# rakhimovv/lvt

Measured on AMD Instinct MI355X. Metric: video-clips/sec/node (VQVAE+DSFVT train step, BAIR 64x64x16), higher is better.
Workload: dtype f32

## Files before the change

include/lvt_hip.h:

```cpp
#ifndef LVT_HIP_H
#define LVT_HIP_H
#include <stddef.h>
#include <stdint.h>
#ifdef __cplusplus
extern "C" {
#endif

#define LVT_OK            0
#define LVT_EINVAL      (-1)
#define LVT_EWORKSPACE  (-2)
#define LVT_ELAUNCH     (-3)
#define LVT_ENODEVICE   (-4)

const char *lvt_last_error(void);
int lvt_version(void);
int lvt_device_info(char *name, int name_len, int *cus, int *clock_khz, long long *hbm_bytes);

#define LVT_MATH_F32   (1 << 16)
#define LVT_MATH_F16X2 (1 << 18)
typedef struct { const float *a; const float *b; float *c; } lvt_amax_io;
int lvt_amax(const float *x, long long n, float *out, void *stream);
typedef struct { const float *x; long long n; float *out; } lvt_amax_entry;
int lvt_amax_multi(const lvt_amax_entry *entries, int n, void *stream);
int lvt_amax_merge(const float *a, const float *b, float *out, void *stream);
#define LVT_VQ_COARSE  (1 << 17)
#define LVT_VQ_GENERIC (1 << 22)

#define LVT_EPI_BIAS        1
#define LVT_EPI_RESIDUAL    2
#define LVT_EPI_RELU        4
#define LVT_EPI_TANH        8
#define LVT_EPI_MASK       16
#define LVT_EPI_ACCUM      32
#define LVT_EPI_PLANES     64
#define LVT_EPI_SIGMOID   128
#define LVT_EPI_PAD(n)    (((n) & 3) << 24)
#define LVT_EPI_PAD_OF(flags) (((flags) >> 24) & 3)
#define LVT_EPI_LEAKY       (1 << 11)
#define LVT_EPI_LEAKY_MASK  (1 << 12)
#define LVT_CAUSAL_KMAX   (1 << 8)
#define LVT_CAUSAL_KMIN   (1 << 9)
#define LVT_CAUSAL_TILE   (1 << 10)

typedef struct {
    int M, N, K;
    int ta, tb;
    const float *A; long long lda; int a_kb; long long a_skb;
    const float *B; long long ldb; int b_kb; long long b_skb;
    float *C;       long long ldc;
    int batch_outer, batch_inner;
    long long sA_o, sA_i, sB_o, sB_i, sC_o, sC_i;
    float alpha;
    int flags;
    const float *bias;
    const float *res;  long long ldr;
    const float *mask; long long ldm;
    int splits;
    float *a_colsum;
    long long c_plane;
    const float *a_amax, *b_amax;
    const float *a_amax2, *b_amax2;
    float *c_amax;
} lvt_gemm_desc;
size_t lvt_gemm_workspace_bytes(const lvt_gemm_desc *d);
int lvt_gemm_f32(const lvt_gemm_desc *d, void *workspace, size_t workspace_bytes, void *stream);

int lvt_vq_argmax_scores(const float *scores, long long rows, int K, long long ld, const float *codebook, int D,
                         long long *idx, void *stream);

typedef struct {
    int M, N, K;
    const void *A; long long lda; int a_planes; int a_kb; long long a_skb;
    const void *B; long long ldb;
    float *C; long long ldc;
    int batch_outer, batch_inner;
    long long sA_o, sA_i, sB_o, sB_i, sC_o, sC_i;
    float alpha;
    int flags;
    const float *bias;
    const float *res;  long long ldr;
    const float *mask; long long ldm;
    const float *a_amax, *b_amax;
    float *c_amax;
    void *Cp; long long ldcp; const float *cp_amax;
} lvt_gemm_p2_desc;
int lvt_gemm_p2_f32(const lvt_gemm_p2_desc *d, void *stream);
typedef struct { const float *src; void *dst; int rows, cols; long long ld_src, ld_dst; int transpose; const float *amax;
                 int batch; long long bs_src, bs_dst; } lvt_p2_pack_entry;
int lvt_p2_pack_multi(const lvt_p2_pack_entry *entries, int n, void *stream);

int lvt_gemm_smallm_f32(int M, int N, int K, int tb, const float *A, long long lda, const float *B,
                        long long ldb, float *C, long long ldc, int batch, long long sB, long long sC,
                        float alpha, int flags, const float *bias, const float *res, long long ldr,
                        const int *pos, long long c_pos, long long r_pos, void *stream);
size_t lvt_gemm_smallm_splitk_workspace_bytes(int M, int N, int splits);
int lvt_gemm_smallm_splitk_f32(int M, int N, int K, int splits, const float *A, long long lda, const float *B,
                               long long ldb, float *C, long long ldc, float alpha, int flags, const float *bias,
                               const float *res, long long ldr, const int *pos, long long c_pos, long long r_pos,
                               void *workspace, size_t workspace_bytes, void *stream);
int lvt_gemm_smallm_partial_f32(int M, int N, int K, int splits, const float *A, long long lda, const float *B,
                                long long ldb, void *workspace, size_t workspace_bytes, void *stream);
int lvt_splitsum_layernorm_fwd(const float *partials, int splits, int rows, int d, const float *bias, const float *res,
                               long long ldr, float *x_out, float eps, const float *w, const float *b, float *y,
                               void *stream);

typedef struct {
    int N, Ti, Hi, Wi, Ci;
    int To, Ho, Wo, Co;
    int Kt, Kh, Kw;
    int st, sh, sw;
    int pt, ph, pw;
} lvt_conv_geom;
int lvt_conv3d_pack_weight(const lvt_conv_geom *g, const float *w, int Ci_real, int Co_real,
                           float *wp, void *stream);
typedef struct { const float *w; float *dst; int kind, taps, Ci, Co, Ci_real, Co_real; } lvt_pack_entry;
int lvt_conv3d_pack_weights_multi(const lvt_pack_entry *entries, int n, void *stream);
#define LVT_CONV_WEIGHT_IMAGE (1 << 21)
typedef struct { const float *wp; int rows, cols; const float *amax; } lvt_weight_image_entry;
size_t lvt_conv3d_weight_image_bytes(int rows, int cols);
int lvt_conv3d_weight_images(const lvt_weight_image_entry *entries, int n, void *stream);
int lvt_conv3d_pack_weight_t(const lvt_conv_geom *g, const float *w, int Ci_real, int Co_real,
                             float *wt, void *stream);
int lvt_conv3d_uses_patch_kernel(const lvt_conv_geom *g, int flags);
int lvt_conv3d_fwd_uses_parity_kernel(const lvt_conv_geom *g, int flags);
int lvt_conv3d_pack_weight_parity(const lvt_conv_geom *g, const float *w, int Ci_real, int Co_real,
                                  float *wq, void *stream);
int lvt_conv3d_fwd_parity(const lvt_conv_geom *g, const float *x, const float *wq, const float *bias,
                          const float *res, const float *mask, float *y, int flags, const lvt_amax_io *ax,
        void *stream);
int lvt_conv3d_fwd(const lvt_conv_geom *g, const float *x, const float *wp, const float *bias,
                   const float *res, const float *mask, float *y, int flags, const lvt_amax_io *ax,
        void *stream);
int lvt_conv3d_bwd_data_uses_phase_kernel(const lvt_conv_geom *g, int flags);
int lvt_conv3d_pack_weight_phases(const lvt_conv_geom *g, const float *w, int Ci_real, int Co_real,
                                  float *wph, void *stream);
int lvt_conv3d_bwd_data_phases(const lvt_conv_geom *g, const float *dy, const float *wph, const float *bias,
                               const float *res, const float *mask, float *dx, int flags, const lvt_amax_io *ax,
        void *stream);
int lvt_conv3d_bwd_data(const lvt_conv_geom *g, const float *dy, const float *wp, const float *bias,
                        const float *res, const float *mask, float *dx, int flags, const lvt_amax_io *ax,
        void *stream);
size_t lvt_conv3d_bwd_weight_workspace_bytes(const lvt_conv_geom *g);
int lvt_conv3d_bwd_weight_fuses_bias(const lvt_conv_geom *g, int flags);
#define LVT_WGRAD_DB_OF_X (1 << 20)
int lvt_conv3d_bwd_weight(const lvt_conv_geom *g, const float *x, const float *dy, float *dw, float *db,
                          int Ci_real, int Co_real, int flags, const lvt_amax_io *ax, void *workspace,
                          size_t workspace_bytes, void *stream);
int lvt_convt4_fwd(const float *x, const float *w, const float *bias, int N, int Hi, int Wi, int Ci, int Cr,
                   int act_tanh, float *y, int flags, const lvt_amax_io *ax, void *stream);
int lvt_convt4_fwd_act(const float *x, const float *w, const float *bias, int N, int Hi, int Wi, int Ci, int Cr,
                       int act, float *y, int flags, const lvt_amax_io *ax, void *stream);
size_t lvt_colsum_workspace_bytes(long long M, int N);
int lvt_colsum(const float *g, long long M, int N, long long ld, float *out, void *workspace,
               size_t workspace_bytes, void *stream);

size_t lvt_vq_nearest_workspace_bytes(long long rows, int num, int KC);
size_t lvt_vq_nearest_generic_workspace_bytes(int num, int D, int KC);
int lvt_vq_nearest(const float *z, long long rows, int ldz, int num, int D, int KC,
                   const float *codebooks, long long *idx, int P, int flags, void *workspace, size_t workspace_bytes,
                   void *stream);
int lvt_vq_gather(const long long *idx, const float *codebooks, long long rows, int num, int D, int KC,
                  int P, float *out, int ldo, void *stream);
size_t lvt_vq_ema_workspace_bytes(long long rows, int num, int D, int KC);
int lvt_vq_ema_accumulate(const long long *idx, const float *z, long long rows, int ldz, int num, int D,
                          int KC, int P, float *stats, void *workspace, size_t workspace_bytes,
                          void *stream);
int lvt_vq_ema_finalize(const float *stats, int num, int D, int KC, float decay, float eps,
                        float *running_size, float *running_sum, float *weight, void *stream);
int lvt_vq_restart_candidates(const float *z, long long rows_local, int ldz, int num, int D, int KC, int P, int rank,
                              int world, unsigned long long seed, const long long *pass, int shared_index, float *cand,
                              void *stream);
int lvt_vq_ema_finalize_restart(const float *stats, const float *cand, int num, int D, int KC, float decay, float eps,
                                float threshold, float *running_size, float *running_sum, float *weight, float *health,
                                long long *restarts_total, long long *pass, void *stream);

int lvt_to_channels_last(const float *in, int B, int C, long long R, int ldo, int mode, const float *a,
                         const float *s, float *out, float *out_amax, void *stream);
int lvt_to_channels_first(const float *in, int B, int C, long long R, int ldi, int mode, const float *a,
                          const float *s, float lo, float hi, float *out, void *stream);

size_t lvt_reduce_workspace_bytes(void);
int lvt_mse_fwd(const float *a, const float *b, long long n, double denom, float scale, float *out,
                void *workspace, size_t workspace_bytes, void *stream);
int lvt_mse_bwd(const float *a, const float *b, long long n, double denom, float scale,
                const float *gout_dev, const float *add, int tanh_of_a, float *out, float *out_amax, void *stream);
int lvt_l1_fwd(const float *a, const float *b, long long n, double denom, float scale, float *out,
               void *workspace, size_t workspace_bytes, void *stream);
int lvt_l1_bwd(const float *a, const float *b, long long n, double denom, float scale,
               const float *gout_dev, const float *add, int tanh_of_a, float *out, float *out_amax, void *stream);
int lvt_tanh_bwd(const float *g, const float *y, long long n, float *out, float *out_amax, void *stream);
int lvt_sigmoid_bwd(const float *g, const float *y, long long n, float *out, float *out_amax, void *stream);
int lvt_axpy(const float *x, const float *add, long long n, const float *alpha_dev, float alpha,
             float *out, void *stream);
int lvt_add_periodic(float *x, const float *table, long long rows, int P, int d, void *stream);

int lvt_layernorm_fwd(const float *x, long long rows, int d, float eps, const float *w, const float *b,
                      float *y, float *mean, float *rstd, float *y_amax, const float *w_amax, const float *b_amax,
                      void *stream);
int lvt_layernorm_fwd_p2(const float *x, long long rows, int d, float eps, const float *w, const float *b,
                         float *y, void *yp, float *mean, float *rstd, float *y_amax, const float *w_amax,
                         const float *b_amax, void *stream);
size_t lvt_layernorm_bwd_workspace_bytes(int d);
int lvt_layernorm_bwd(const float *dy, const float *x, const float *mean, const float *rstd,
                      const float *w, long long rows, int d, const float *add, float *dx, float *dw,
                      float *db, float *dx_amax, void *workspace, size_t workspace_bytes, void *stream);

int lvt_attn_softmax_fwd(float *scores, int B, int H, int S, float temper, const float *dt,
                         const float *dh, const float *dw, int bt, int bh, int bw, int masked, float fill,
                         void *stream);
int lvt_attn_softmax_bwd(const float *P, float *dP, int B, int H, int S, float temper, int bt, int bh,
                         int bw, float *G, float *ddt, float *ddh, float *ddw, void *stream);

int lvt_attn_fwd(const float *q, const float *k, const float *v, int B, int H, int S, int da, float temper,
                 const float *dt, const float *dh, const float *dw, int bt, int bh, int bw, int masked, float fill,
                 float *P, float *o, void *stream);

int lvt_attn_planes_supported(int S, int da, int bt, int bh, int bw);
int lvt_attn_fwd_planes(const void *qkv_planes, long long plane_stride, long long operand_stride, int B, int H, int S, int da,
                        float temper, const float *dt, const float *dh, const float *dw, int bt, int bh, int bw, int masked,
                        float fill, float *P, float *o, float *o_amax, void *stream);
size_t lvt_attn_bwd_planes_workspace_bytes(int B, int H, int S, int bt, int bh, int bw);
int lvt_attn_bwd_planes(const void *qkv_planes, long long plane_stride, long long operand_stride, const void *do_planes,
                        const float *P, const float *o, int B, int H, int S, int da, float temper, int bt, int bh, int bw,
                        int masked, float *dq, float *dk, float *dv, float *ddt, float *ddh, float *ddw, float *d_amax,
                        void *workspace, size_t workspace_bytes, void *stream);

int lvt_attn_flash_supported(int S, int da, int bt, int bh, int bw);
int lvt_attn_fwd_flash(const float *q, const float *k, const float *v, long long ld, int B, int H, int S, int da,
                       float temper, const float *dt, const float *dh, const float *dw, int bt, int bh, int bw,
                       int masked, float fill, float *o, float *stats, float *o_amax, void *stream);
size_t lvt_attn_bwd_flash_workspace_bytes(int B, int H, int S, int bt, int bh, int bw);
int lvt_attn_bwd_flash(const float *q, const float *k, const float *v, const float *d_o, long long ld, const float *stats,
                       const float *o, int B, int H, int S, int da, float temper, const float *dt, const float *dh, const float *dw,
                       int bt, int bh, int bw, int masked, float fill, float *dq, float *dk, float *dv, float *ddt,
                       float *ddh, float *ddw, float *d_amax, void *workspace, size_t workspace_bytes, void *stream);

int lvt_attn_decode(const float *q, long long ldq, const float *Kc, const float *Vc, int B, int H, int S, int da, int qi,
                    float temper, const float *dt, const float *dh, const float *dw, int bt, int bh, int bw,
                    float *o, const int *pos, long long q_pos, void *stream);
int lvt_attn_decode_blocks(const float *q, long long ldq, const float *Kc, const float *Vc, int B, int H, int da, int qi,
                           float temper, const float *dt, const float *dh, const float *dw, int st, int sh, int sw,
                           int bt, int bh, int bw, float *o, const int *pos, long long q_pos, void *stream);

int lvt_decode_gather_codes(const long long *codes, const long long *nb, const int *pos, int rows, int S1, int taps,
                            long long *out, void *stream);
int lvt_decode_commit(const long long *drawn, int rows, int S1, long long *codes, int *pos, void *stream);

int lvt_sample_categorical(const float *logits, long long rows, int V, float temp, const float *u,
                           long long *out, long long out_stride, float *probs, const int *pos, long long u_pos,
                           void *stream);

int lvt_embbag_fwd(const long long *idx, long long bstride, int P, long long rows, int nslots,
                   const int *slot_off, const int *tab_row, const float *table, int D, const float *bias,
                   const float *btable, const long long *bindex, float *out, void *stream);
#define LVT_ONEHOT_DENSE (1 << 19)
size_t lvt_onehot_tn_workspace_bytes(int nslots, int V, int N, long long rows);
int lvt_onehot_tn_is_gather(int nslots, int V, int N, long long ldb, const float *dout, int flags);
int lvt_onehot_tn_gemm(const long long *idx, int nslots, int V, const int *slot_off, long long bstride,
                       long long pstride, int P, long long rows, const float *dout, long long ldb, int N,
                       float *out, int flags, const float *dout_amax, void *workspace, size_t workspace_bytes,
                       void *stream);
int lvt_permute3(const float *in, long long s0, long long s1, long long s2, int n0, int n1, int n2,
                 float *out, void *stream);

int lvt_row_gather(const float *x, const long long *perm, long long B, int S, int d, float *out, void *stream);

int lvt_slice_context(const long long *video, int B, int T, int nc, int H, int W, const int *abc, int st, int sh,
                      int sw, int kt, int kh, int kw, int n_prime, long long pad_value, long long *ctx,
                      long long *slice, long long *slice_idx, unsigned char *ignore, void *stream);

size_t lvt_xent_workspace_bytes(void);
int lvt_xent_fwd(const float *logits, const long long *target, long long tstride_b, long long tstride_pos,
                 int P, long long rows, int V, long long ignore, float scale, float *row_loss, float *lse,
                 float *loss, float *count, void *workspace, size_t workspace_bytes, void *stream);
int lvt_xent_bwd(const float *logits, const long long *target, long long tstride_b, long long tstride_pos,
                 int P, long long rows, int V, long long ignore, const float *lse, const float *count,
                 const float *gout, float scale, float *dlogits, float *dl_amax, void *stream);

typedef struct {
    float *p; const float *g; float *s0; float *s1;
    long long n; float lr; float wd;
} lvt_opt_entry;
int lvt_adam_step(const lvt_opt_entry *entries, int n, float beta1, float beta2, float eps, int step,
                  void *stream);
int lvt_rmsprop_step(const lvt_opt_entry *entries, int n, float alpha, float eps, float momentum,
                     void *stream);

typedef struct { const float *g; long long n; } lvt_grad_entry;
typedef struct {
    float norm;
    float coef;
    int skip;
    int reserved;
} lvt_clip_record;
long long lvt_grad_sqnorm_partials(const lvt_grad_entry *entries, int n);
int lvt_grad_sqnorm(const lvt_grad_entry *entries, int n, double *partials, long long n_partials, void *stream);
int lvt_grad_clip_coef(const double *partials, long long n_partials, float max_norm, lvt_clip_record *record,
                       long long *skipped, void *stream);
int lvt_adam_step_scaled(const lvt_opt_entry *entries, int n, float beta1, float beta2, float eps, int step,
                         const lvt_clip_record *gscale, float clamp, void *stream);
int lvt_rmsprop_step_scaled(const lvt_opt_entry *entries, int n, float alpha, float eps, float momentum,
                            const lvt_clip_record *gscale, float clamp, void *stream);

#define LVT_BN_RUNNING  1
#define LVT_BN_UPDATE   2
#define LVT_BN_UNBIASED 4
#define LVT_BN_COUNT    8
#define LVT_BN_TRAIN    16
size_t lvt_bn_workspace_bytes(long long M, int Cp);
int lvt_bn_stats(const float *y, long long M, int Cp, float *stats, void *workspace, size_t workspace_bytes, void *stream);
int lvt_bn_finalize(const float *stats, int nranks, long long count, int C, int Cp, const float *gamma, const float *beta,
                    float *running_mean, float *running_var, long long *num_batches_tracked, float momentum, float eps,
                    int flags, float *scale, float *shift, float *saved, void *stream);
int lvt_bn_apply(const float *y, const float *res, long long M, int Cp, const float *scale, const float *shift, int flags,
                 float *out, float *out_amax, void *stream);
int lvt_bn_bwd_reduce(const float *g, const float *y, long long M, int Cp, const float *saved, float *sums, void *workspace,
                      size_t workspace_bytes, void *stream);
int lvt_bn_bwd_apply(const float *g, const float *y, long long M, int Cp, const float *scale, const float *saved,
                     const float *sums, long long n, int flags, float *dy, float *dy_amax, void *stream);
typedef struct {
    const float *w; float *w_out; int outer, Co, inner, Cp;
    const float *gamma, *beta, *running_mean, *running_var; float eps;
    float *bias_out; float *w_amax;
} lvt_bn_fold_entry;
int lvt_bn_fold(const lvt_bn_fold_entry *entries, int n, void *stream);


int lvt_pool2x2(const float *x, int N, int H, int W, int Cp, float scale, const float *mask, int mask_flags, float *out,
                float *out_amax, void *stream);
int lvt_upsample2x2(const float *x, int N, int H, int W, int Cp, float scale, const float *mask, int mask_flags, float *out,
                    float *out_amax, void *stream);

int lvt_pixel_shuffle2(const float *x, int N, int H, int W, int C, int act, float *out, float *out_amax, void *stream);
int lvt_pixel_unshuffle2(const float *g, int N, int H, int W, int C, float *out, float *out_amax, void *stream);

#ifdef __cplusplus
}
#endif
#endif
```

lvt_amd/csrc/elementwise.hip:

```cpp
#include "lvt_common.h"

static inline int grid_for(long long n, int per_block, int cap = 8192) {
    long long b = lvt_cdiv(n, per_block);
    if (b < 1) b = 1;
    return (int)(b < cap ? b : cap);
}

__device__ __forceinline__ float wave_sum(float v) {
#pragma unroll
    for (int off = 32; off >= 1; off >>= 1) v += __shfl_xor(v, off);
    return v;
}
__device__ __forceinline__ float wave_max(float v) {
#pragma unroll
    for (int off = 32; off >= 1; off >>= 1) v = fmaxf(v, __shfl_xor(v, off));
    return v;
}

__global__ void lvt_to_channels_last_kernel(const float *__restrict__ in, int B, int C, long long R, int ldo,
                                            int mode, const float *__restrict__ a, const float *__restrict__ s,
                                            float *__restrict__ out, float *__restrict__ out_amax) {
    __shared__ float amax_scratch[4];
    float am = 0.f;
    const long long total = (long long)B * R * ldo;
    for (long long i = (long long)blockIdx.x * blockDim.x + threadIdx.x; i < total;
         i += (long long)gridDim.x * blockDim.x) {
        const int c = i % ldo; const long long t = i / ldo;
        const long long r = t % R; const long long b = t / R;
        float v = 0.f;
        if (c < C) {
            v = in[(b * C + c) * R + r];
            if (mode == 1) v = (v - a[c]) / s[c];
        }
        out[i] = v;
        am = fmaxf(am, lvt_absf(v));
    }
    if (out_amax) lvt_block_amax_commit(am, out_amax, amax_scratch);
}
__global__ void lvt_to_channels_first_kernel(const float *__restrict__ in, int B, int C, long long R, int ldi,
                                             int mode, const float *__restrict__ a, const float *__restrict__ s,
                                             float lo, float hi, float *__restrict__ out) {
    const long long total = (long long)B * C * R;
    for (long long i = (long long)blockIdx.x * blockDim.x + threadIdx.x; i < total;
         i += (long long)gridDim.x * blockDim.x) {
        const long long r = i % R; const long long t = i / R;
        const int c = t % C; const long long b = t / C;
        float v = in[(b * R + r) * ldi + c];
        if (mode == 2) { v = v * s[c] + a[c]; v = fminf(fmaxf(v, lo), hi); }
        out[i] = v;
    }
}

extern "C" int lvt_to_channels_last(const float *in, int B, int C, long long R, int ldo, int mode, const float *a,
                                    const float *s, float *out, float *out_amax, void *stream) {
    LVT_REQUIRE(in && out && B > 0 && C > 0 && R > 0 && ldo >= C, "to_channels_last: bad args");
    LVT_REQUIRE(mode == 0 || (a && s), "to_channels_last: affine tables missing");
    hipLaunchKernelGGL(lvt_to_channels_last_kernel, dim3(grid_for((long long)B * R * ldo, 256, out_amax ? 2048 : 8192)), dim3(256), 0,
                       (hipStream_t)stream, in, B, C, R, ldo, mode, a, s, out, out_amax);
    LVT_CHECK_LAUNCH("lvt_to_channels_last_kernel");
    return LVT_OK;
}
extern "C" int lvt_to_channels_first(const float *in, int B, int C, long long R, int ldi, int mode, const float *a,
                                     const float *s, float lo, float hi, float *out, void *stream) {
    LVT_REQUIRE(in && out && B > 0 && C > 0 && R > 0 && ldi >= C, "to_channels_first: bad args");
    LVT_REQUIRE(mode == 0 || (a && s), "to_channels_first: affine tables missing");
    hipLaunchKernelGGL(lvt_to_channels_first_kernel, dim3(grid_for((long long)B * C * R, 256)), dim3(256), 0,
                       (hipStream_t)stream, in, B, C, R, ldi, mode, a, s, lo, hi, out);
    LVT_CHECK_LAUNCH("lvt_to_channels_first_kernel");
    return LVT_OK;
}

#define RED_BLOCKS 1024
template <int L1>
__global__ void lvt_sqdiff_partial_kernel(const float *__restrict__ a, const float *__restrict__ b, long long n4,
                                          float *__restrict__ partial) {
    __shared__ float red[256];
    float s = 0.f;
    for (long long i = (long long)blockIdx.x * blockDim.x + threadIdx.x; i < n4;
         i += (long long)gridDim.x * blockDim.x) {
        const float4 x = reinterpret_cast<const float4 *>(a)[i];
        const float4 y = reinterpret_cast<const float4 *>(b)[i];
        const float d0 = x.x - y.x, d1 = x.y - y.y, d2 = x.z - y.z, d3 = x.w - y.w;
        if (L1) s += (fabsf(d0) + fabsf(d1)) + (fabsf(d2) + fabsf(d3));
        else s += (d0 * d0 + d1 * d1) + (d2 * d2 + d3 * d3);
    }
    red[threadIdx.x] = s;
    __syncthreads();
    for (int k = 128; k > 0; k >>= 1) {
        if (threadIdx.x < k) red[threadIdx.x] += red[threadIdx.x + k];
        __syncthreads();
    }
    if (threadIdx.x == 0) partial[blockIdx.x] = red[0];
}
__global__ void lvt_scalar_finish_kernel(const float *__restrict__ partial, int n, float scale,
                                         const float *__restrict__ denom_dev, float *__restrict__ out) {
    __shared__ double red[256];
    double s = 0.0;
    for (int i = threadIdx.x; i < n; i += 256) s += (double)partial[i];
    red[threadIdx.x] = s;
    __syncthreads();
    for (int k = 128; k > 0; k >>= 1) {
        if (threadIdx.x < k) red[threadIdx.x] += red[threadIdx.x + k];
        __syncthreads();
    }
    if (threadIdx.x == 0) {
        double v = red[0] * (double)scale;
        if (denom_dev) v /= (double)fmaxf(denom_dev[0], 1.0f);
        out[0] = (float)v;
    }
}
extern "C" size_t lvt_reduce_workspace_bytes(void) { return (size_t)RED_BLOCKS * sizeof(float) * 2; }

extern "C" int lvt_mse_fwd(const float *a, const float *b, long long n, double denom, float scale, float *out,
                           void *workspace, size_t workspace_bytes, void *stream) {
    LVT_REQUIRE(a && b && out && n > 0 && n % 4 == 0 && denom > 0, "mse_fwd: bad args");
    LVT_REQUIRE(workspace && workspace_bytes >= lvt_reduce_workspace_bytes(), "mse_fwd: workspace");
    hipStream_t s = (hipStream_t)stream;
    const int blocks = grid_for(n / 4, 256 * 4, RED_BLOCKS);
    hipLaunchKernelGGL(lvt_sqdiff_partial_kernel<0>, dim3(blocks), dim3(256), 0, s, a, b, n / 4, (float *)workspace);
    LVT_CHECK_LAUNCH("lvt_sqdiff_partial_kernel");
    hipLaunchKernelGGL(lvt_scalar_finish_kernel, dim3(1), dim3(256), 0, s, (const float *)workspace, blocks,
                       (float)((double)scale / denom), (const float *)nullptr, out);
    LVT_CHECK_LAUNCH("lvt_scalar_finish_kernel");
    return LVT_OK;
}
extern "C" int lvt_l1_fwd(const float *a, const float *b, long long n, double denom, float scale, float *out,
                          void *workspace, size_t workspace_bytes, void *stream) {
    LVT_REQUIRE(a && b && out && n > 0 && n % 4 == 0 && denom > 0, "l1_fwd: bad args");
    LVT_REQUIRE(workspace && workspace_bytes >= lvt_reduce_workspace_bytes(), "l1_fwd: workspace");
    hipStream_t s = (hipStream_t)stream;
    const int blocks = grid_for(n / 4, 256 * 4, RED_BLOCKS);
    hipLaunchKernelGGL(lvt_sqdiff_partial_kernel<1>, dim3(blocks), dim3(256), 0, s, a, b, n / 4, (float *)workspace);
    LVT_CHECK_LAUNCH("lvt_sqdiff_partial_kernel<l1>");
    hipLaunchKernelGGL(lvt_scalar_finish_kernel, dim3(1), dim3(256), 0, s, (const float *)workspace, blocks,
                       (float)((double)scale / denom), (const float *)nullptr, out);
    LVT_CHECK_LAUNCH("lvt_scalar_finish_kernel");
    return LVT_OK;
}

template <int L1>
__global__ void lvt_mse_bwd_kernel(const float *__restrict__ a, const float *__restrict__ b, long long n4, float c,
                                   const float *__restrict__ gout, const float *__restrict__ add, int tanh_of_a,
                                   float *__restrict__ out, float *__restrict__ out_amax) {
    __shared__ float amax_scratch[4];
    float am = 0.f;
    const float g = (gout ? gout[0] : 1.0f) * c;
    for (long long i = (long long)blockIdx.x * blockDim.x + threadIdx.x; i < n4;
         i += (long long)gridDim.x * blockDim.x) {
        const float4 x = reinterpret_cast<const float4 *>(a)[i];
        const float4 y = reinterpret_cast<const float4 *>(b)[i];
        float4 r = make_float4(x.x - y.x, x.y - y.y, x.z - y.z, x.w - y.w);
        if (L1) r = make_float4((float)((r.x > 0.f) - (r.x < 0.f)), (float)((r.y > 0.f) - (r.y < 0.f)), (float)((r.z > 0.f) - (r.z < 0.f)),
                                (float)((r.w > 0.f) - (r.w < 0.f)));
        r.x *= g; r.y *= g; r.z *= g; r.w *= g;
        if (tanh_of_a) {
            r.x *= 1.f - x.x * x.x; r.y *= 1.f - x.y * x.y; r.z *= 1.f - x.z * x.z; r.w *= 1.f - x.w * x.w;
        }
        if (add) {
            const float4 z = reinterpret_cast<const float4 *>(add)[i];
            r.x += z.x; r.y += z.y; r.z += z.z; r.w += z.w;
        }
        reinterpret_cast<float4 *>(out)[i] = r;
        am = fmaxf(am, fmaxf(fmaxf(lvt_absf(r.x), lvt_absf(r.y)), fmaxf(lvt_absf(r.z), lvt_absf(r.w))));
    }
    if (out_amax) lvt_block_amax_commit(am, out_amax, amax_scratch);
}
extern "C" int lvt_mse_bwd(const float *a, const float *b, long long n, double denom, float scale,
                           const float *gout_dev, const float *add, int tanh_of_a, float *out, float *out_amax, void *stream) {
    LVT_REQUIRE(a && b && out && n > 0 && n % 4 == 0 && denom > 0, "mse_bwd: bad args");
    hipLaunchKernelGGL(lvt_mse_bwd_kernel<0>, dim3(grid_for(n / 4, 256, out_amax ? 2048 : 8192)), dim3(256), 0, (hipStream_t)stream, a, b,
                       n / 4, (float)(2.0 * (double)scale / denom), gout_dev, add, tanh_of_a, out, out_amax);
    LVT_CHECK_LAUNCH("lvt_mse_bwd_kernel");
    return LVT_OK;
}
extern "C" int lvt_l1_bwd(const float *a, const float *b, long long n, double denom, float scale,
                          const float *gout_dev, const float *add, int tanh_of_a, float *out, float *out_amax, void *stream) {
    LVT_REQUIRE(a && b && out && n > 0 && n % 4 == 0 && denom > 0, "l1_bwd: bad args");
    hipLaunchKernelGGL(lvt_mse_bwd_kernel<1>, dim3(grid_for(n / 4, 256, out_amax ? 2048 : 8192)), dim3(256), 0, (hipStream_t)stream, a, b,
                       n / 4, (float)((double)scale / denom), gout_dev, add, tanh_of_a, out, out_amax);
    LVT_CHECK_LAUNCH("lvt_mse_bwd_kernel<l1>");
    return LVT_OK;
}

__global__ void lvt_axpy_kernel(const float *__restrict__ x, const float *__restrict__ add, long long n,
                                const float *__restrict__ alpha_dev, float alpha, float *__restrict__ out) {
    const float a = alpha * (alpha_dev ? alpha_dev[0] : 1.0f);
    for (long long i = (long long)blockIdx.x * blockDim.x + threadIdx.x; i < n;
         i += (long long)gridDim.x * blockDim.x)
        out[i] = a * x[i] + (add ? add[i] : 0.f);
}
extern "C" int lvt_axpy(const float *x, const float *add, long long n, const float *alpha_dev, float alpha,
                        float *out, void *stream) {
    LVT_REQUIRE(x && out && n > 0, "axpy: bad args");
    hipLaunchKernelGGL(lvt_axpy_kernel, dim3(grid_for(n, 256)), dim3(256), 0, (hipStream_t)stream, x, add, n,
                       alpha_dev, alpha, out);
    LVT_CHECK_LAUNCH("lvt_axpy_kernel");
    return LVT_OK;
}

__global__ void lvt_tanh_bwd_kernel(const float *__restrict__ g, const float *__restrict__ y, long long n4,
                                    float *__restrict__ out, float *__restrict__ out_amax) {
    __shared__ float amax_scratch[4];
    float am = 0.f;
    for (long long i = (long long)blockIdx.x * blockDim.x + threadIdx.x; i < n4;
         i += (long long)gridDim.x * blockDim.x) {
        const float4 a = reinterpret_cast<const float4 *>(g)[i];
        const float4 t = reinterpret_cast<const float4 *>(y)[i];
        const float4 r = make_float4(a.x * (1.f - t.x * t.x), a.y * (1.f - t.y * t.y), a.z * (1.f - t.z * t.z), a.w * (1.f - t.w * t.w));
        reinterpret_cast<float4 *>(out)[i] = r;
        am = fmaxf(am, fmaxf(fmaxf(lvt_absf(r.x), lvt_absf(r.y)), fmaxf(lvt_absf(r.z), lvt_absf(r.w))));
    }
    if (out_amax) lvt_block_amax_commit(am, out_amax, amax_scratch);
}
extern "C" int lvt_tanh_bwd(const float *g, const float *y, long long n, float *out, float *out_amax, void *stream) {
    LVT_REQUIRE(g && y && out && n > 0 && n % 4 == 0, "tanh_bwd: bad args");
    hipLaunchKernelGGL(lvt_tanh_bwd_kernel, dim3(grid_for(n / 4, 256, out_amax ? 2048 : 8192)), dim3(256), 0, (hipStream_t)stream, g, y,
                       n / 4, out, out_amax);
    LVT_CHECK_LAUNCH("lvt_tanh_bwd_kernel");
    return LVT_OK;
}

__global__ void lvt_sigmoid_bwd_kernel(const float *__restrict__ g, const float *__restrict__ y, long long n4,
                                       float *__restrict__ out, float *__restrict__ out_amax) {
    __shared__ float amax_scratch[4];
    float am = 0.f;
    for (long long i = (long long)blockIdx.x * blockDim.x + threadIdx.x; i < n4;
         i += (long long)gridDim.x * blockDim.x) {
        const float4 a = reinterpret_cast<const float4 *>(g)[i];
        const float4 t = reinterpret_cast<const float4 *>(y)[i];
        const float4 r = make_float4(a.x * (t.x * (1.f - t.x)), a.y * (t.y * (1.f - t.y)), a.z * (t.z * (1.f - t.z)), a.w * (t.w * (1.f - t.w)));
        reinterpret_cast<float4 *>(out)[i] = r;
        am = fmaxf(am, fmaxf(fmaxf(lvt_absf(r.x), lvt_absf(r.y)), fmaxf(lvt_absf(r.z), lvt_absf(r.w))));
    }
    if (out_amax) lvt_block_amax_commit(am, out_amax, amax_scratch);
}
extern "C" int lvt_sigmoid_bwd(const float *g, const float *y, long long n, float *out, float *out_amax, void *stream) {
    LVT_REQUIRE(g && y && out && n > 0 && n % 4 == 0, "sigmoid_bwd: bad args");
    hipLaunchKernelGGL(lvt_sigmoid_bwd_kernel, dim3(grid_for(n / 4, 256, out_amax ? 2048 : 8192)), dim3(256), 0, (hipStream_t)stream, g, y,
                       n / 4, out, out_amax);
    LVT_CHECK_LAUNCH("lvt_sigmoid_bwd_kernel");
    return LVT_OK;
}

__global__ void lvt_add_periodic_kernel(float *__restrict__ x, const float *__restrict__ table, long long rows,
                                        int P, int d4) {
    const long long total = rows * d4;
    for (long long i = (long long)blockIdx.x * blockDim.x + threadIdx.x; i < total;
         i += (long long)gridDim.x * blockDim.x) {
        const long long r = i / d4; const int c = i % d4;
        float4 v = reinterpret_cast<float4 *>(x)[i];
        const float4 t = reinterpret_cast<const float4 *>(table)[(r % P) * d4 + c];
        v.x += t.x; v.y += t.y; v.z += t.z; v.w += t.w;
        reinterpret_cast<float4 *>(x)[i] = v;
    }
}
extern "C" int lvt_add_periodic(float *x, const float *table, long long rows, int P, int d, void *stream) {
    LVT_REQUIRE(x && table && rows > 0 && P > 0 && d % 4 == 0, "add_periodic: bad args");
    hipLaunchKernelGGL(lvt_add_periodic_kernel, dim3(grid_for(rows * (d / 4), 256)), dim3(256), 0,
                       (hipStream_t)stream, x, table, rows, P, d / 4);
    LVT_CHECK_LAUNCH("lvt_add_periodic_kernel");
    return LVT_OK;
}

#define LN_MAXV 4
__device__ __forceinline__ float ln_bound(const float *w_amax, const float *b_amax, int d) {
    return fmaf(*w_amax, sqrtf((float)(d - 1)), *b_amax) * (1.0f + 0x1p-20f);
}
__device__ __forceinline__ float ln_mix_lo(unsigned h, float k, float c) {
    float r;
    asm("v_fma_mix_f32 %0, %1, %2, %3 op_sel:[0,0,0] op_sel_hi:[1,0,0]" : "=v"(r) : "v"(h), "v"(k), "v"(c));
    return r;
}
__device__ __forceinline__ float ln_mix_hi(unsigned h, float k, float c) {
    float r;
    asm("v_fma_mix_f32 %0, %1, %2, %3 op_sel:[1,0,0] op_sel_hi:[1,0,0]" : "=v"(r) : "v"(h), "v"(k), "v"(c));
    return r;
}
typedef float ln_f32x2 __attribute__((ext_vector_type(2)));
typedef _Float16 ln_f16x2 __attribute__((ext_vector_type(2)));
__device__ __forceinline__ void ln_split_pair(float a, float b, float s, unsigned &ph, unsigned &pl) {
    const ln_f32x2 v = {a, b};
    ph = __builtin_bit_cast(unsigned, __builtin_convertvector(v * s, ln_f16x2));
    const ln_f32x2 t2 = v * (s * 2048.f);
    const ln_f32x2 r = {ln_mix_lo(ph, -2048.f, t2.x), ln_mix_hi(ph, -2048.f, t2.y)};
    pl = __builtin_bit_cast(unsigned, __builtin_convertvector(r, ln_f16x2));
}
template <int P2>
__global__ void lvt_layernorm_fwd_kernel(const float *__restrict__ x, long long rows, int d, float eps,
                                         const float *__restrict__ w, const float *__restrict__ b,
                                         float *__restrict__ y, float *__restrict__ mean_out,
                                         float *__restrict__ rstd_out, float *__restrict__ y_amax,
                                         const float *__restrict__ w_amax, const float *__restrict__ b_amax,
                                         char *__restrict__ yimg) {
    __shared__ float amax_scratch[4];
    const int lane = threadIdx.x & 63;
    const int d4 = d / 4;
    float am = 0.f;
    float ps = 1.f;
    if (P2) {
        int un = 0;
        ps = lvt_f16_scale_bits(__float_as_uint(ln_bound(w_amax, b_amax, d)), un);
    }
    if (y_amax && w_amax) {
        if (blockIdx.x == 0 && threadIdx.x == 0) *y_amax = ln_bound(w_amax, b_amax, d);
        y_amax = nullptr;
    }
    for (long long row = ((long long)blockIdx.x * blockDim.x + threadIdx.x) >> 6; row < rows;
         row += ((long long)gridDim.x * blockDim.x) >> 6) {
        const float4 *xp = reinterpret_cast<const float4 *>(x + row * d);
        float4 v[LN_MAXV];
        float s = 0.f;
#pragma unroll
        for (int i = 0; i < LN_MAXV; ++i) {
            const int c = lane + 64 * i;
            v[i] = c < d4 ? xp[c] : make_float4(0.f, 0.f, 0.f, 0.f);
            s += (v[i].x + v[i].y) + (v[i].z + v[i].w);
        }
        const float mean = wave_sum(s) / d;
        float q = 0.f;
#pragma unroll
        for (int i = 0; i < LN_MAXV; ++i) {
            if (lane + 64 * i < d4) {
                const float a0 = v[i].x - mean, a1 = v[i].y - mean, a2 = v[i].z - mean, a3 = v[i].w - mean;
                q += (a0 * a0 + a1 * a1) + (a2 * a2 + a3 * a3);
            }
        }
        const float rstd = 1.0f / sqrtf(wave_sum(q) / d + eps);
        float4 *yp = reinterpret_cast<float4 *>(y + row * d);
#pragma unroll
        for (int i = 0; i < LN_MAXV; ++i) {
            const int c = lane + 64 * i;
            if (c < d4) {
                const float4 ww = reinterpret_cast<const float4 *>(w)[c];
                const float4 bb = reinterpret_cast<const float4 *>(b)[c];
                float4 o;
                o.x = (v[i].x - mean) * rstd * ww.x + bb.x; o.y = (v[i].y - mean) * rstd * ww.y + bb.y;
                o.z = (v[i].z - mean) * rstd * ww.z + bb.z; o.w = (v[i].w - mean) * rstd * ww.w + bb.w;
                yp[c] = o;
                if (P2) {
                    uint2 ph, pl;
                    ln_split_pair(o.x, o.y, ps, ph.x, pl.x);
                    ln_split_pair(o.z, o.w, ps, ph.y, pl.y);
                    char *ip = yimg + (long long)row * d * 4 + (c >> 3) * 128 + (c & 7) * 8;
                    *reinterpret_cast<uint2 *>(ip) = ph;
                    *reinterpret_cast<uint2 *>(ip + 64) = pl;
                }
                am = fmaxf(am, fmaxf(fmaxf(lvt_absf(o.x), lvt_absf(o.y)), fmaxf(lvt_absf(o.z), lvt_absf(o.w))));
            }
        }
        if (lane == 0 && mean_out) { mean_out[row] = mean; rstd_out[row] = rstd; }
    }
    if (y_amax) lvt_block_amax_commit(am, y_amax, amax_scratch);
}
#define LN_FWD_MAX_BLOCKS 16384
extern "C" int lvt_layernorm_fwd(const float *x, long long rows, int d, float eps, const float *w, const float *b,
                                 float *y, float *mean, float *rstd, float *y_amax, const float *w_amax, const float *b_amax,
                                 void *stream) {
    LVT_REQUIRE(x && w && b && y && rows > 0 && d % 4 == 0 && d <= 256 * LN_MAXV, "layernorm_fwd: bad args (d=%d)", d);
    LVT_REQUIRE(!w_amax == !b_amax, "layernorm_fwd: w_amax and b_amax come together");
    hipLaunchKernelGGL(lvt_layernorm_fwd_kernel<0>, dim3(grid_for(rows, 4, (y_amax && !w_amax) ? 2048 : LN_FWD_MAX_BLOCKS)), dim3(256), 0,
                       (hipStream_t)stream, x, rows, d, eps, w, b, y, mean, rstd, y_amax, w_amax, b_amax, (char *)nullptr);
    LVT_CHECK_LAUNCH("lvt_layernorm_fwd_kernel");
    return LVT_OK;
}
extern "C" int lvt_layernorm_fwd_p2(const float *x, long long rows, int d, float eps, const float *w, const float *b,
                                    float *y, void *yp, float *mean, float *rstd, float *y_amax, const float *w_amax,
                                    const float *b_amax, void *stream) {
    LVT_REQUIRE(x && w && b && y && yp && rows > 0 && d % 32 == 0 && d <= 256 * LN_MAXV, "layernorm_fwd_p2: bad args (d=%d)", d);
    LVT_REQUIRE(y_amax && w_amax && b_amax, "layernorm_fwd_p2: the image is scaled by the a-priori bound: y_amax, w_amax, b_amax are required");
    LVT_REQUIRE(((uintptr_t)yp & 127) == 0, "layernorm_fwd_p2: the image must be 128-byte aligned");
    hipLaunchKernelGGL(lvt_layernorm_fwd_kernel<1>, dim3(grid_for(rows, 4, LN_FWD_MAX_BLOCKS)), dim3(256), 0,
                       (hipStream_t)stream, x, rows, d, eps, w, b, y, mean, rstd, y_amax, w_amax, b_amax, (char *)yp);
    LVT_CHECK_LAUNCH("lvt_layernorm_fwd_kernel<p2>");
    return LVT_OK;
}

#define LN_BWD_BLOCKS 512
#define LN_BWD_ROWS 1
__global__ __launch_bounds__(256) void lvt_layernorm_bwd_kernel(
    const float *__restrict__ dy, const float *__restrict__ x, const float *__restrict__ mean,
    const float *__restrict__ rstd, const float *__restrict__ w, long long rows, int d, const float *__restrict__ add,
    float *__restrict__ dx, float *__restrict__ pdw, float *__restrict__ pdb, float *__restrict__ dx_amax) {
    __shared__ float amax_scratch[4];
    float am = 0.f;
    __shared__ float sdw[4][256 * LN_MAXV];
    __shared__ float sdb[4][256 * LN_MAXV];
    const int lane = threadIdx.x & 63, wave = threadIdx.x >> 6;
    const int d4 = d / 4;
    float4 adw[LN_MAXV], adb[LN_MAXV];
#pragma unroll
    for (int i = 0; i < LN_MAXV; ++i) { adw[i] = make_float4(0.f, 0.f, 0.f, 0.f); adb[i] = adw[i]; }
    const long long rows_per_block = lvt_cdiv(rows, gridDim.x);
    const long long r0 = blockIdx.x * rows_per_block;
    const long long r1 = min(rows, r0 + rows_per_block);
    for (long long row0 = r0 + wave; row0 < r1; row0 += 4 * LN_BWD_ROWS) {
        float4 xh[LN_BWD_ROWS][LN_MAXV], gw[LN_BWD_ROWS][LN_MAXV], zv[LN_BWD_ROWS][LN_MAXV];
        float rs[LN_BWD_ROWS], s1[LN_BWD_ROWS], s2[LN_BWD_ROWS];
#pragma unroll
        for (int u = 0; u < LN_BWD_ROWS; ++u) {
            const long long row = row0 + 4 * u;
            if (row >= r1) continue;
            if (add) {
#pragma unroll
                for (int i = 0; i < LN_MAXV; ++i)
                    if (lane + 64 * i < d4) zv[u][i] = reinterpret_cast<const float4 *>(add + row * d)[lane + 64 * i];
            }
            const float m = mean[row];
            rs[u] = rstd[row];
            const float4 *xp = reinterpret_cast<const float4 *>(x + row * d);
            const float4 *gp = reinterpret_cast<const float4 *>(dy + row * d);
            s1[u] = 0.f; s2[u] = 0.f;
#pragma unroll
            for (int i = 0; i < LN_MAXV; ++i) {
                const int c = lane + 64 * i;
                if (c < d4) {
                    const float4 xv = xp[c], gv = gp[c], ww = reinterpret_cast<const float4 *>(w)[c];
                    const float r = rs[u];
                    xh[u][i] = make_float4((xv.x - m) * r, (xv.y - m) * r, (xv.z - m) * r, (xv.w - m) * r);
                    gw[u][i] = make_float4(gv.x * ww.x, gv.y * ww.y, gv.z * ww.z, gv.w * ww.w);
                    const float4 h = xh[u][i], g = gw[u][i];
                    s1[u] += (g.x + g.y) + (g.z + g.w);
                    s2[u] += (g.x * h.x + g.y * h.y) + (g.z * h.z + g.w * h.w);
                    adw[i].x += gv.x * h.x; adw[i].y += gv.y * h.y; adw[i].z += gv.z * h.z; adw[i].w += gv.w * h.w;
                    adb[i].x += gv.x; adb[i].y += gv.y; adb[i].z += gv.z; adb[i].w += gv.w;
                }
            }
        }
#pragma unroll
        for (int u = 0; u < LN_BWD_ROWS; ++u) {
            const long long row = row0 + 4 * u;
            if (row >= r1) continue;
            const float m1 = wave_sum(s1[u]) / d, m2 = wave_sum(s2[u]) / d;
            float4 *op = reinterpret_cast<float4 *>(dx + row * d);
#pragma unroll
            for (int i = 0; i < LN_MAXV; ++i) {
                const int c = lane + 64 * i;
                if (c < d4) {
                    const float4 h = xh[u][i], g = gw[u][i];
                    const float r = rs[u];
                    float4 o;
                    o.x = r * (g.x - m1 - h.x * m2); o.y = r * (g.y - m1 - h.y * m2);
                    o.z = r * (g.z - m1 - h.z * m2); o.w = r * (g.w - m1 - h.w * m2);
                    if (add) {
                        const float4 z = zv[u][i];
                        o.x += z.x; o.y += z.y; o.z += z.z; o.w += z.w;
                    }
                    op[c] = o;
                    am = fmaxf(am, fmaxf(fmaxf(lvt_absf(o.x), lvt_absf(o.y)), fmaxf(lvt_absf(o.z), lvt_absf(o.w))));
                }
            }
        }
    }
    if (dx_amax) lvt_block_amax_commit(am, dx_amax, amax_scratch);
#pragma unroll
    for (int i = 0; i < LN_MAXV; ++i) {
        const int c = lane + 64 * i;
        if (c < d4) {
            reinterpret_cast<float4 *>(sdw[wave])[c] = adw[i];
            reinterpret_cast<float4 *>(sdb[wave])[c] = adb[i];
        }
    }
    __syncthreads();
    for (int c = threadIdx.x; c < d; c += 256) {
        pdw[(long long)blockIdx.x * d + c] = ((sdw[0][c] + sdw[1][c]) + sdw[2][c]) + sdw[3][c];
        pdb[(long long)blockIdx.x * d + c] = ((sdb[0][c] + sdb[1][c]) + sdb[2][c]) + sdb[3][c];
    }
}
__global__ __launch_bounds__(256) void lvt_rowsum_partials_kernel(const float *__restrict__ partial0, const float *__restrict__ partial1,
                                                                  int nblk, int n, float *__restrict__ out0, float *__restrict__ out1) {
    __shared__ float red[256];
    const float *partial = blockIdx.y ? partial1 : partial0;
    float *out = blockIdx.y ? out1 : out0;
    constexpr int cols = 8, RL = 256 / cols;
    const int c = blockIdx.x * cols + (threadIdx.x % cols);
    const int rl = threadIdx.x / cols;
    float s0 = 0.f, s1 = 0.f, s2 = 0.f, s3 = 0.f;
    if (c < n) {
        int b = rl;
        for (; b + 3 * RL < nblk; b += 4 * RL) {
            s0 += partial[(long long)b * n + c]; s1 += partial[(long long)(b + RL) * n + c];
            s2 += partial[(long long)(b + 2 * RL) * n + c]; s3 += partial[(long long)(b + 3 * RL) * n + c];
        }
        for (; b < nblk; b += RL) s0 += partial[(long long)b * n + c];
    }
    float s = (s0 + s1) + (s2 + s3);
    red[threadIdx.x] = s;
    __syncthreads();
    if (rl == 0 && c < n) {
        for (int k = 1; k < RL; ++k) s += red[k * cols + threadIdx.x];
        out[c] = s;
    }
}
extern "C" size_t lvt_layernorm_bwd_workspace_bytes(int d) { return (size_t)2 * LN_BWD_BLOCKS * d * sizeof(float); }
extern "C" int lvt_layernorm_bwd(const float *dy, const float *x, const float *mean, const float *rstd,
                                 const float *w, long long rows, int d, const float *add, float *dx, float *dw,
                                 float *db, float *dx_amax, void *workspace, size_t workspace_bytes, void *stream) {
    LVT_REQUIRE(dy && x && mean && rstd && w && dx && dw && db && rows > 0 && d % 4 == 0 && d <= 256 * LN_MAXV,
                "layernorm_bwd: bad args");
    LVT_REQUIRE(workspace && workspace_bytes >= lvt_layernorm_bwd_workspace_bytes(d), "layernorm_bwd: workspace");
    hipStream_t s = (hipStream_t)stream;
    int blocks = (int)(lvt_cdiv(rows, 8) < LN_BWD_BLOCKS ? lvt_cdiv(rows, 8) : LN_BWD_BLOCKS);
    const long long rpb = lvt_cdiv(rows, blocks);
    blocks = (int)lvt_cdiv(rows, rpb);
    float *pdw = (float *)workspace, *pdb = pdw + (size_t)LN_BWD_BLOCKS * d;
    hipLaunchKernelGGL(lvt_layernorm_bwd_kernel, dim3(blocks), dim3(256), 0, s, dy, x, mean, rstd, w, rows, d, add,
                       dx, pdw, pdb, dx_amax);
    LVT_CHECK_LAUNCH("lvt_layernorm_bwd_kernel");
    hipLaunchKernelGGL(lvt_rowsum_partials_kernel, dim3((d + 7) / 8, 2), dim3(256), 0, s, (const float *)pdw, (const float *)pdb,
                       blocks, d, dw, db);
    LVT_CHECK_LAUNCH("lvt_rowsum_partials_kernel");
    return LVT_OK;
}

struct SliceGeom { int B, T, nc, H, W, st, sh, sw, kt, kh, kw, n_prime, t, h, w, Tc, Hc, Wc; long long pad; };
__global__ void lvt_slice_context_kernel(const long long *__restrict__ video, const int *__restrict__ abc, SliceGeom g,
                                         long long *__restrict__ ctx, long long *__restrict__ slice,
                                         long long *__restrict__ slice_idx, unsigned char *__restrict__ ignore) {
    const long long n_ctx = (long long)g.B * g.nc * g.Tc * g.Hc * g.Wc;
    const long long n_sl = (long long)g.B * g.nc * g.t * g.h * g.w;
    const long long n_ig = (long long)g.B * g.t * g.h * g.w;
    const long long total = n_ctx + n_sl + n_ig + g.B;
    for (long long i = (long long)blockIdx.x * blockDim.x + threadIdx.x; i < total; i += (long long)gridDim.x * blockDim.x) {
        if (i < n_ctx) {
            long long r = i;
            const int ow = r % g.Wc; r /= g.Wc;
            const int oh = r % g.Hc; r /= g.Hc;
            const int ot = r % g.Tc; r /= g.Tc;
            const int ch = r % g.nc; const int b = r / g.nc;
            const int a = abc[3 * b], bo = abc[3 * b + 1], c = abc[3 * b + 2];
            const int ti = ot - g.kt / 2 + a, hi = oh - g.kh / 2 + bo, wi = ow - g.kw / 2 + c;
            long long v = g.pad;
            if ((unsigned)ti < (unsigned)g.T && (unsigned)hi < (unsigned)g.H && (unsigned)wi < (unsigned)g.W) {
                const int mine = ((ti % g.st) * g.sh + (hi % g.sh)) * g.sw + (wi % g.sw);
                if (mine < (a * g.sh + bo) * g.sw + c)
                    v = video[((((long long)b * g.T + ti) * g.nc + ch) * g.H + hi) * g.W + wi];
            }
            ctx[i] = v;
        } else if (i < n_ctx + n_sl) {
            long long r = i - n_ctx;
            const int wi = r % g.w; r /= g.w;
            const int hi = r % g.h; r /= g.h;
            const int ti = r % g.t; r /= g.t;
            const int ch = r % g.nc; const int b = r / g.nc;
            const int a = abc[3 * b], bo = abc[3 * b + 1], c = abc[3 * b + 2];
            slice[i - n_ctx] = video[((((long long)b * g.T + ti * g.st + a) * g.nc + ch) * g.H + hi * g.sh + bo) * g.W + wi * g.sw + c];
        } else if (i < n_ctx + n_sl + n_ig) {
            long long r = i - n_ctx - n_sl;
            r /= (long long)g.h * g.w;
            const int ti = r % g.t; const int b = r / g.t;
            ignore[i - n_ctx - n_sl] = (ti * g.st + abc[3 * b]) < g.n_prime ? 1 : 0;
        } else {
            const int b = (int)(i - n_ctx - n_sl - n_ig);
            slice_idx[b] = (abc[3 * b] * g.sh + abc[3 * b + 1]) * g.sw + abc[3 * b + 2];
        }
    }
}
extern "C" int lvt_slice_context(const long long *video, int B, int T, int nc, int H, int W, const int *abc, int st, int sh,
                                 int sw, int kt, int kh, int kw, int n_prime, long long pad_value, long long *ctx,
                                 long long *slice, long long *slice_idx, unsigned char *ignore, void *stream) {
    LVT_REQUIRE(video && abc && ctx && slice && slice_idx && ignore, "slice_context: null pointer");
    LVT_REQUIRE(B > 0 && nc > 0 && st > 0 && sh > 0 && sw > 0 && T % st == 0 && H % sh == 0 && W % sw == 0 &&
                kt > 0 && kh > 0 && kw > 0, "slice_context: bad geometry");
    SliceGeom g;
    g.B = B; g.T = T; g.nc = nc; g.H = H; g.W = W; g.st = st; g.sh = sh; g.sw = sw; g.kt = kt; g.kh = kh; g.kw = kw;
    g.n_prime = n_prime; g.pad = pad_value;
    g.t = T / st; g.h = H / sh; g.w = W / sw;
    g.Tc = 2 * (kt / 2) + (g.t - 1) * st + 1; g.Hc = 2 * (kh / 2) + (g.h - 1) * sh + 1; g.Wc = 2 * (kw / 2) + (g.w - 1) * sw + 1;
    const long long total = (long long)B * nc * g.Tc * g.Hc * g.Wc + (long long)B * (nc + 1) * g.t * g.h * g.w + B;
    const int blocks = (int)(lvt_cdiv(total, 256) < 4096 ? lvt_cdiv(total, 256) : 4096);
    hipLaunchKernelGGL(lvt_slice_context_kernel, dim3(blocks), dim3(256), 0, (hipStream_t)stream, video, abc, g, ctx, slice,
                       slice_idx, ignore);
    LVT_CHECK_LAUNCH("lvt_slice_context_kernel");
    return LVT_OK;
}

__global__ void lvt_row_gather_kernel(const float *__restrict__ x, const long long *__restrict__ perm, long long B, int S,
                                      int d4, float *__restrict__ out) {
    const long long total = B * S * d4;
    for (long long i = (long long)blockIdx.x * blockDim.x + threadIdx.x; i < total; i += (long long)gridDim.x * blockDim.x) {
        const int c = i % d4; const long long r = i / d4;
        const int s = r % S; const long long b = r / S;
        reinterpret_cast<float4 *>(out)[i] = reinterpret_cast<const float4 *>(x)[(b * S + perm[s]) * d4 + c];
    }
}
extern "C" int lvt_row_gather(const float *x, const long long *perm, long long B, int S, int d, float *out, void *stream) {
    LVT_REQUIRE(x && perm && out && B > 0 && S > 0 && d > 0 && d % 4 == 0 && lvt_aligned16(x) && lvt_aligned16(out),
                "row_gather: bad args");
    const long long total = B * S * (d / 4);
    const int blocks = (int)(lvt_cdiv(total, 256) < 8192 ? lvt_cdiv(total, 256) : 8192);
    hipLaunchKernelGGL(lvt_row_gather_kernel, dim3(blocks), dim3(256), 0, (hipStream_t)stream, x, perm, B, S, d / 4, out);
    LVT_CHECK_LAUNCH("lvt_row_gather_kernel");
    return LVT_OK;
}

__global__ __launch_bounds__(256) void lvt_amax_kernel(const float *__restrict__ x, long long n, float *__restrict__ out) {
    __shared__ float scratch[4];
    const long long n4 = n >> 2;
    float m = 0.f;
    if ((((uintptr_t)x) & 15) == 0) {
        float m1 = 0.f;
        long long i = (long long)blockIdx.x * blockDim.x + threadIdx.x;
        const long long step = (long long)gridDim.x * blockDim.x;
        for (; i + step < n4; i += 2 * step) {
            const float4 v = *reinterpret_cast<const float4 *>(x + i * 4), u = *reinterpret_cast<const float4 *>(x + (i + step) * 4);
            m = fmaxf(m, fmaxf(fmaxf(lvt_absf(v.x), lvt_absf(v.y)), fmaxf(lvt_absf(v.z), lvt_absf(v.w))));
            m1 = fmaxf(m1, fmaxf(fmaxf(lvt_absf(u.x), lvt_absf(u.y)), fmaxf(lvt_absf(u.z), lvt_absf(u.w))));
        }
        if (i < n4) {
            const float4 v = *reinterpret_cast<const float4 *>(x + i * 4);
            m = fmaxf(m, fmaxf(fmaxf(lvt_absf(v.x), lvt_absf(v.y)), fmaxf(lvt_absf(v.z), lvt_absf(v.w))));
        }
        m = fmaxf(m, m1);
        for (long long t = n4 * 4 + (long long)blockIdx.x * blockDim.x + threadIdx.x; t < n; t += step) m = fmaxf(m, lvt_absf(x[t]));
    } else {
        for (long long i = (long long)blockIdx.x * blockDim.x + threadIdx.x; i < n; i += (long long)gridDim.x * blockDim.x)
            m = fmaxf(m, lvt_absf(x[i]));
    }
    lvt_block_amax_commit(m, out, scratch);
}
struct AmaxTable { const float *x[64]; long long n[64]; float *out[64]; };
__global__ __launch_bounds__(256) void lvt_amax_multi_kernel(const AmaxTable t) {
    __shared__ float scratch[4];
    const float *x = t.x[blockIdx.y];
    const long long n = t.n[blockIdx.y], n4 = (((uintptr_t)x) & 15) == 0 ? n >> 2 : 0;
    float m = 0.f;
    for (long long i = (long long)blockIdx.x * blockDim.x + threadIdx.x; i < n4; i += (long long)gridDim.x * blockDim.x) {
        const float4 v = *reinterpret_cast<const float4 *>(x + i * 4);
        m = fmaxf(m, fmaxf(fmaxf(lvt_absf(v.x), lvt_absf(v.y)), fmaxf(lvt_absf(v.z), lvt_absf(v.w))));
    }
    for (long long i = n4 * 4 + (long long)blockIdx.x * blockDim.x + threadIdx.x; i < n; i += (long long)gridDim.x * blockDim.x)
        m = fmaxf(m, lvt_absf(x[i]));
    lvt_block_amax_commit(m, t.out[blockIdx.y], scratch);
}
extern "C" int lvt_amax_multi(const lvt_amax_entry *entries, int n, void *stream) {
    LVT_REQUIRE(entries && n > 0, "amax_multi: bad args");
    for (int base = 0; base < n; base += 64) {
        const int cnt = n - base < 64 ? n - base : 64;
        AmaxTable t;
        long long biggest = 0;
        for (int i = 0; i < cnt; ++i) {
            const lvt_amax_entry &e = entries[base + i];
            LVT_REQUIRE(e.x && e.out && e.n > 0, "amax_multi: bad entry %d", base + i);
            t.x[i] = e.x; t.n[i] = e.n; t.out[i] = e.out;
            if (e.n > biggest) biggest = e.n;
        }
        hipLaunchKernelGGL(lvt_amax_multi_kernel, dim3(grid_for(biggest / 4 + 1, 256 * 4, 64), cnt), dim3(256), 0, (hipStream_t)stream, t);
        LVT_CHECK_LAUNCH("lvt_amax_multi_kernel");
    }
    return LVT_OK;
}
__global__ void lvt_amax_merge_kernel(const float *a, const float *b, float *out) {
    float m = fmaxf(*out, *a);
    if (b) m = fmaxf(m, *b);
    *out = m;
}
extern "C" int lvt_amax_merge(const float *a, const float *b, float *out, void *stream) {
    LVT_REQUIRE(a && out, "amax_merge: bad args");
    hipLaunchKernelGGL(lvt_amax_merge_kernel, dim3(1), dim3(1), 0, (hipStream_t)stream, a, b, out);
    LVT_CHECK_LAUNCH("lvt_amax_merge_kernel");
    return LVT_OK;
}
extern "C" int lvt_amax(const float *x, long long n, float *out, void *stream) {
    LVT_REQUIRE(x && out && n > 0, "amax: bad args");
    hipLaunchKernelGGL(lvt_amax_kernel, dim3(grid_for(n / 4 + 1, 256 * 8, 1024)), dim3(256), 0, (hipStream_t)stream, x, n, out);
    LVT_CHECK_LAUNCH("lvt_amax_kernel");
    return LVT_OK;
}
```

lvt_amd/hip/binding.py:

```python
import ctypes as C
import os

import torch

_HERE = os.path.dirname(os.path.abspath(__file__))
_LIB_PATH = os.environ.get("LVT_HIP_LIB") or os.path.join(os.path.dirname(_HERE), "liblvt_hip.so")

EPI_BIAS, EPI_RESIDUAL, EPI_RELU, EPI_TANH, EPI_MASK, EPI_ACCUM, EPI_PLANES = 1, 2, 4, 8, 16, 32, 64
EPI_SIGMOID = 128
EPI_LEAKY, EPI_LEAKY_MASK = 1 << 11, 1 << 12


def epi_pad(n):
    if not 0 <= n <= 3:
        raise ValueError("epi_pad: 0..3 pad channels, got %r" % (n,))
    return n << 24
CAUSAL_KMAX, CAUSAL_KMIN, CAUSAL_TILE = 1 << 8, 1 << 9, 1 << 10
ABI_VERSION = 680
MATH_F32 = 1 << 16
MATH_F16X2 = 1 << 18
ONEHOT_DENSE = 1 << 19
WGRAD_DB_OF_X = 1 << 20
CONV_WEIGHT_IMAGE = 1 << 21
BN_RUNNING, BN_UPDATE, BN_UNBIASED, BN_COUNT, BN_TRAIN = 1, 2, 4, 8, 16


class LvtError(RuntimeError):
    pass


class GemmDesc(C.Structure):
    _fields_ = [
        ("M", C.c_int), ("N", C.c_int), ("K", C.c_int), ("ta", C.c_int), ("tb", C.c_int),
        ("A", C.c_void_p), ("lda", C.c_longlong), ("a_kb", C.c_int), ("a_skb", C.c_longlong),
        ("B", C.c_void_p), ("ldb", C.c_longlong), ("b_kb", C.c_int), ("b_skb", C.c_longlong),
        ("C", C.c_void_p), ("ldc", C.c_longlong),
        ("batch_outer", C.c_int), ("batch_inner", C.c_int),
        ("sA_o", C.c_longlong), ("sA_i", C.c_longlong), ("sB_o", C.c_longlong), ("sB_i", C.c_longlong),
        ("sC_o", C.c_longlong), ("sC_i", C.c_longlong),
        ("alpha", C.c_float), ("flags", C.c_int),
        ("bias", C.c_void_p), ("res", C.c_void_p), ("ldr", C.c_longlong),
        ("mask", C.c_void_p), ("ldm", C.c_longlong), ("splits", C.c_int),
        ("a_colsum", C.c_void_p), ("c_plane", C.c_longlong),
        ("a_amax", C.c_void_p), ("b_amax", C.c_void_p), ("a_amax2", C.c_void_p), ("b_amax2", C.c_void_p), ("c_amax", C.c_void_p),
    ]


class GemmP2Desc(C.Structure):
    _fields_ = [
        ("M", C.c_int), ("N", C.c_int), ("K", C.c_int),
        ("A", C.c_void_p), ("lda", C.c_longlong), ("a_planes", C.c_int), ("a_kb", C.c_int), ("a_skb", C.c_longlong),
        ("B", C.c_void_p), ("ldb", C.c_longlong),
        ("C", C.c_void_p), ("ldc", C.c_longlong),
        ("batch_outer", C.c_int), ("batch_inner", C.c_int),
        ("sA_o", C.c_longlong), ("sA_i", C.c_longlong), ("sB_o", C.c_longlong), ("sB_i", C.c_longlong),
        ("sC_o", C.c_longlong), ("sC_i", C.c_longlong),
        ("alpha", C.c_float), ("flags", C.c_int),
        ("bias", C.c_void_p), ("res", C.c_void_p), ("ldr", C.c_longlong),
        ("mask", C.c_void_p), ("ldm", C.c_longlong),
        ("a_amax", C.c_void_p), ("b_amax", C.c_void_p), ("c_amax", C.c_void_p),
        ("Cp", C.c_void_p), ("ldcp", C.c_longlong), ("cp_amax", C.c_void_p),
    ]


class P2PackEntry(C.Structure):
    _fields_ = [("src", C.c_void_p), ("dst", C.c_void_p), ("rows", C.c_int), ("cols", C.c_int), ("ld_src", C.c_longlong),
                ("ld_dst", C.c_longlong), ("transpose", C.c_int), ("amax", C.c_void_p),
                ("batch", C.c_int), ("bs_src", C.c_longlong), ("bs_dst", C.c_longlong)]


class AmaxEntry(C.Structure):
    _fields_ = [("x", C.c_void_p), ("n", C.c_longlong), ("out", C.c_void_p)]


class PackEntry(C.Structure):
    _fields_ = [("w", C.c_void_p), ("dst", C.c_void_p), ("kind", C.c_int), ("taps", C.c_int), ("Ci", C.c_int), ("Co", C.c_int),
                ("Ci_real", C.c_int), ("Co_real", C.c_int)]


class WeightImageEntry(C.Structure):
    _fields_ = [("wp", C.c_void_p), ("rows", C.c_int), ("cols", C.c_int), ("amax", C.c_void_p)]


class BnFoldEntry(C.Structure):
    _fields_ = [("w", C.c_void_p), ("w_out", C.c_void_p), ("outer", C.c_int), ("Co", C.c_int), ("inner", C.c_int),
                ("Cp", C.c_int), ("gamma", C.c_void_p), ("beta", C.c_void_p), ("running_mean", C.c_void_p),
                ("running_var", C.c_void_p), ("eps", C.c_float), ("bias_out", C.c_void_p), ("w_amax", C.c_void_p)]


class AmaxIO(C.Structure):
    _fields_ = [("a", C.c_void_p), ("b", C.c_void_p), ("c", C.c_void_p)]


class OptEntry(C.Structure):
    _fields_ = [("p", C.c_void_p), ("g", C.c_void_p), ("s0", C.c_void_p), ("s1", C.c_void_p),
                ("n", C.c_longlong), ("lr", C.c_float), ("wd", C.c_float)]


class GradEntry(C.Structure):
    _fields_ = [("g", C.c_void_p), ("n", C.c_longlong)]


CLIP_RECORD_BYTES = 16


class ConvGeom(C.Structure):
    _fields_ = [(n, C.c_int) for n in
                ("N", "Ti", "Hi", "Wi", "Ci", "To", "Ho", "Wo", "Co", "Kt", "Kh", "Kw",
                 "st", "sh", "sw", "pt", "ph", "pw")]

    def key(self):
        return tuple(getattr(self, n) for n, _ in self._fields_)


_lib = None


def _declare(lib):
    vp, ci, cll, cf, sz = C.c_void_p, C.c_int, C.c_longlong, C.c_float, C.c_size_t
    P = C.POINTER
    sigs = {
        "lvt_last_error": (C.c_char_p, []),
        "lvt_version": (ci, []),
        "lvt_device_info": (ci, [C.c_char_p, ci, P(ci), P(ci), P(cll)]),
        "lvt_gemm_workspace_bytes": (sz, [P(GemmDesc)]),
        "lvt_gemm_f32": (ci, [P(GemmDesc), vp, sz, vp]),
        "lvt_vq_argmax_scores": (ci, [vp, cll, ci, cll, vp, ci, vp, vp]),
        "lvt_gemm_p2_f32": (ci, [P(GemmP2Desc), vp]),
        "lvt_p2_pack_multi": (ci, [P(P2PackEntry), ci, vp]),
        "lvt_layernorm_fwd_p2": (ci, [vp, cll, ci, cf, vp, vp, vp, vp, vp, vp, vp, vp, vp, vp]),
        "lvt_gemm_smallm_f32": (ci, [ci, ci, ci, ci, vp, cll, vp, cll, vp, cll, ci, cll, cll, cf, ci, vp, vp, cll, vp, cll, cll, vp]),
        "lvt_gemm_smallm_splitk_workspace_bytes": (sz, [ci, ci, ci]),
        "lvt_gemm_smallm_splitk_f32": (ci, [ci, ci, ci, ci, vp, cll, vp, cll, vp, cll, cf, ci, vp, vp, cll, vp, cll, cll, vp, sz, vp]),
        "lvt_gemm_smallm_partial_f32": (ci, [ci, ci, ci, ci, vp, cll, vp, cll, vp, sz, vp]),
        "lvt_splitsum_layernorm_fwd": (ci, [vp, ci, ci, ci, vp, vp, cll, vp, cf, vp, vp, vp, vp]),
        "lvt_conv3d_pack_weight": (ci, [P(ConvGeom), vp, ci, ci, vp, vp]),
        "lvt_conv3d_pack_weight_t": (ci, [P(ConvGeom), vp, ci, ci, vp, vp]),
        "lvt_conv3d_uses_patch_kernel": (ci, [P(ConvGeom), ci]),
        "lvt_conv3d_fwd_uses_parity_kernel": (ci, [P(ConvGeom), ci]),
        "lvt_conv3d_pack_weight_parity": (ci, [P(ConvGeom), vp, ci, ci, vp, vp]),
        "lvt_amax": (ci, [vp, cll, vp, vp]),
        "lvt_amax_multi": (ci, [P(AmaxEntry), ci, vp]),
        "lvt_conv3d_pack_weights_multi": (ci, [P(PackEntry), ci, vp]),
        "lvt_conv3d_weight_image_bytes": (sz, [ci, ci]),
        "lvt_conv3d_weight_images": (ci, [P(WeightImageEntry), ci, vp]),
        "lvt_amax_merge": (ci, [vp, vp, vp, vp]),
        "lvt_conv3d_fwd_parity": (ci, [P(ConvGeom), vp, vp, vp, vp, vp, vp, ci, P(AmaxIO), vp]),
        "lvt_conv3d_fwd": (ci, [P(ConvGeom), vp, vp, vp, vp, vp, vp, ci, P(AmaxIO), vp]),
        "lvt_conv3d_bwd_data_uses_phase_kernel": (ci, [P(ConvGeom), ci]),
        "lvt_conv3d_pack_weight_phases": (ci, [P(ConvGeom), vp, ci, ci, vp, vp]),
        "lvt_conv3d_bwd_data_phases": (ci, [P(ConvGeom), vp, vp, vp, vp, vp, vp, ci, P(AmaxIO), vp]),
        "lvt_conv3d_bwd_data": (ci, [P(ConvGeom), vp, vp, vp, vp, vp, vp, ci, P(AmaxIO), vp]),
        "lvt_conv3d_bwd_weight_workspace_bytes": (sz, [P(ConvGeom)]),
        "lvt_conv3d_bwd_weight_fuses_bias": (ci, [P(ConvGeom), ci]),
        "lvt_conv3d_bwd_weight": (ci, [P(ConvGeom), vp, vp, vp, vp, ci, ci, ci, P(AmaxIO), vp, sz, vp]),
        "lvt_convt4_fwd": (ci, [vp, vp, vp, ci, ci, ci, ci, ci, ci, vp, ci, vp, vp]),
        "lvt_convt4_fwd_act": (ci, [vp, vp, vp, ci, ci, ci, ci, ci, ci, vp, ci, vp, vp]),
        "lvt_colsum_workspace_bytes": (sz, [cll, ci]),
        "lvt_colsum": (ci, [vp, cll, ci, cll, vp, vp, sz, vp]),
        "lvt_vq_nearest_workspace_bytes": (sz, [cll, ci, ci]),
        "lvt_vq_nearest_generic_workspace_bytes": (sz, [ci, ci, ci]),
        "lvt_vq_nearest": (ci, [vp, cll, ci, ci, ci, ci, vp, vp, ci, ci, vp, sz, vp]),
        "lvt_vq_gather": (ci, [vp, vp, cll, ci, ci, ci, ci, vp, ci, vp]),
        "lvt_vq_ema_workspace_bytes": (sz, [cll, ci, ci, ci]),
        "lvt_vq_ema_accumulate": (ci, [vp, vp, cll, ci, ci, ci, ci, ci, vp, vp, sz, vp]),
        "lvt_vq_ema_finalize": (ci, [vp, ci, ci, ci, cf, cf, vp, vp, vp, vp]),
        "lvt_vq_restart_candidates": (ci, [vp, cll, ci, ci, ci, ci, ci, ci, ci, C.c_ulonglong, vp, ci, vp, vp]),
        "lvt_vq_ema_finalize_restart": (ci, [vp, vp, ci, ci, ci, cf, cf, cf, vp, vp, vp, vp, vp, vp, vp]),
        "lvt_to_channels_last": (ci, [vp, ci, ci, cll, ci, ci, vp, vp, vp, vp, vp]),
        "lvt_to_channels_first": (ci, [vp, ci, ci, cll, ci, ci, vp, vp, cf, cf, vp, vp]),
        "lvt_reduce_workspace_bytes": (sz, []),
        "lvt_mse_fwd": (ci, [vp, vp, cll, C.c_double, cf, vp, vp, sz, vp]),
        "lvt_mse_bwd": (ci, [vp, vp, cll, C.c_double, cf, vp, vp, ci, vp, vp, vp]),
        "lvt_l1_fwd": (ci, [vp, vp, cll, C.c_double, cf, vp, vp, sz, vp]),
        "lvt_l1_bwd": (ci, [vp, vp, cll, C.c_double, cf, vp, vp, ci, vp, vp, vp]),
        "lvt_tanh_bwd": (ci, [vp, vp, cll, vp, vp, vp]),
        "lvt_sigmoid_bwd": (ci, [vp, vp, cll, vp, vp, vp]),
        "lvt_axpy": (ci, [vp, vp, cll, vp, cf, vp, vp]),
        "lvt_add_periodic": (ci, [vp, vp, cll, ci, ci, vp]),
        "lvt_layernorm_fwd": (ci, [vp, cll, ci, cf, vp, vp, vp, vp, vp, vp, vp, vp, vp]),
        "lvt_layernorm_bwd_workspace_bytes": (sz, [ci]),
        "lvt_layernorm_bwd": (ci, [vp, vp, vp, vp, vp, cll, ci, vp, vp, vp, vp, vp, vp, sz, vp]),
        "lvt_attn_softmax_fwd": (ci, [vp, ci, ci, ci, cf, vp, vp, vp, ci, ci, ci, ci, cf, vp]),
        "lvt_attn_softmax_bwd": (ci, [vp, vp, ci, ci, ci, cf, ci, ci, ci, vp, vp, vp, vp, vp]),
        "lvt_attn_fwd": (ci, [vp, vp, vp, ci, ci, ci, ci, cf, vp, vp, vp, ci, ci, ci, ci, cf, vp, vp, vp]),
        "lvt_attn_planes_supported": (ci, [ci, ci, ci, ci, ci]),
        "lvt_attn_fwd_planes": (ci, [vp, cll, cll, ci, ci, ci, ci, cf, vp, vp, vp, ci, ci, ci, ci, cf, vp, vp, vp, vp]),
        "lvt_attn_bwd_planes_workspace_bytes": (sz, [ci, ci, ci, ci, ci, ci]),
        "lvt_attn_bwd_planes": (ci, [vp, cll, cll, vp, vp, vp, ci, ci, ci, ci, cf, ci, ci, ci, ci, vp, vp, vp, vp, vp, vp, vp, vp, sz, vp]),
        "lvt_attn_flash_supported": (ci, [ci, ci, ci, ci, ci]),
        "lvt_attn_fwd_flash": (ci, [vp, vp, vp, cll, ci, ci, ci, ci, cf, vp, vp, vp, ci, ci, ci, ci, cf, vp, vp, vp, vp]),
        "lvt_attn_bwd_flash_workspace_bytes": (sz, [ci, ci, ci, ci, ci, ci]),
        "lvt_attn_bwd_flash": (ci, [vp, vp, vp, vp, cll, vp, vp, ci, ci, ci, ci, cf, vp, vp, vp, ci, ci, ci, ci, cf, vp, vp, vp, vp,
                                    vp, vp, vp, vp, sz, vp]),
        "lvt_attn_decode": (ci, [vp, cll, vp, vp, ci, ci, ci, ci, ci, cf, vp, vp, vp, ci, ci, ci, vp, vp, cll, vp]),
        "lvt_attn_decode_blocks": (ci, [vp, cll, vp, vp, ci, ci, ci, ci, cf, vp, vp, vp, ci, ci, ci, ci, ci, ci, vp, vp, cll, vp]),
        "lvt_decode_gather_codes": (ci, [vp, vp, vp, ci, ci, ci, vp, vp]),
        "lvt_decode_commit": (ci, [vp, ci, ci, vp, vp, vp]),
        "lvt_sample_categorical": (ci, [vp, cll, ci, cf, vp, vp, cll, vp, vp, cll, vp]),
        "lvt_embbag_fwd": (ci, [vp, cll, ci, cll, ci, P(ci), P(ci), vp, ci, vp, vp, vp, vp, vp]),
        "lvt_onehot_tn_workspace_bytes": (sz, [ci, ci, ci, cll]),
        "lvt_onehot_tn_is_gather": (ci, [ci, ci, ci, cll, vp, ci]),
        "lvt_onehot_tn_gemm": (ci, [vp, ci, ci, P(ci), cll, cll, ci, cll, vp, cll, ci, vp, ci, vp, vp, sz, vp]),
        "lvt_permute3": (ci, [vp, cll, cll, cll, ci, ci, ci, vp, vp]),
        "lvt_row_gather": (ci, [vp, vp, cll, ci, ci, vp, vp]),
        "lvt_slice_context": (ci, [vp, ci, ci, ci, ci, ci, vp, ci, ci, ci, ci, ci, ci, ci, cll, vp, vp, vp, vp, vp]),
        "lvt_xent_workspace_bytes": (sz, []),
        "lvt_xent_fwd": (ci, [vp, vp, cll, cll, ci, cll, ci, cll, cf, vp, vp, vp, vp, vp, sz, vp]),
        "lvt_xent_bwd": (ci, [vp, vp, cll, cll, ci, cll, ci, cll, vp, vp, vp, cf, vp, vp, vp]),
        "lvt_adam_step": (ci, [P(OptEntry), ci, cf, cf, cf, ci, vp]),
        "lvt_rmsprop_step": (ci, [P(OptEntry), ci, cf, cf, cf, vp]),
        "lvt_adam_step_scaled": (ci, [P(OptEntry), ci, cf, cf, cf, ci, vp, cf, vp]),
        "lvt_rmsprop_step_scaled": (ci, [P(OptEntry), ci, cf, cf, cf, vp, cf, vp]),
        "lvt_grad_sqnorm_partials": (cll, [P(GradEntry), ci]),
        "lvt_grad_sqnorm": (ci, [P(GradEntry), ci, vp, cll, vp]),
        "lvt_grad_clip_coef": (ci, [vp, cll, cf, vp, vp, vp]),
        "lvt_bn_workspace_bytes": (sz, [cll, ci]),
        "lvt_bn_stats": (ci, [vp, cll, ci, vp, vp, sz, vp]),
        "lvt_bn_finalize": (ci, [vp, ci, cll, ci, ci, vp, vp, vp, vp, vp, cf, cf, ci, vp, vp, vp, vp]),
        "lvt_bn_apply": (ci, [vp, vp, cll, ci, vp, vp, ci, vp, vp, vp]),
        "lvt_bn_bwd_reduce": (ci, [vp, vp, cll, ci, vp, vp, vp, sz, vp]),
        "lvt_bn_bwd_apply": (ci, [vp, vp, cll, ci, vp, vp, vp, cll, ci, vp, vp, vp]),
        "lvt_bn_fold": (ci, [P(BnFoldEntry), ci, vp]),
        "lvt_pool2x2": (ci, [vp, ci, ci, ci, ci, cf, vp, ci, vp, vp, vp]),
        "lvt_upsample2x2": (ci, [vp, ci, ci, ci, ci, cf, vp, ci, vp, vp, vp]),
        "lvt_pixel_shuffle2": (ci, [vp, ci, ci, ci, ci, ci, vp, vp, vp]),
        "lvt_pixel_unshuffle2": (ci, [vp, ci, ci, ci, ci, vp, vp, vp]),
    }
    for name, (res, args) in sigs.items():
        fn = getattr(lib, name)
        fn.restype = res
        fn.argtypes = args
    return sigs


def available():
    return os.path.exists(_LIB_PATH)


def lib():
    global _lib
    if _lib is None:
        if not os.path.exists(_LIB_PATH):
            raise LvtError("liblvt_hip.so not found at %s -- run `python -c 'import __graft_entry__ as g; "
                           "g.build()'` (or `make -C lvt_amd/csrc`); there is no CPU fallback" % _LIB_PATH)
        handle = C.CDLL(_LIB_PATH)
        handle.lvt_version.restype = C.c_int
        if handle.lvt_version() != ABI_VERSION:
            raise LvtError("liblvt_hip.so at %s has ABI version %d, this package binds version %d -- rebuild it "
                           "(`make -C lvt_amd/csrc`)" % (_LIB_PATH, handle.lvt_version(), ABI_VERSION))
        handle._lvt_sigs = _declare(handle)
        _lib = handle
    return _lib


MATH_MODES = ("f32", "bf16x3", "f16x2")
_math_mode = os.environ.get("LVT_MATH", "f16x2")
if _math_mode not in MATH_MODES:
    raise LvtError("LVT_MATH must be one of %s (got %r)" % (MATH_MODES, _math_mode))


def set_math_mode(mode):
    global _math_mode
    if mode not in MATH_MODES:
        raise LvtError("math mode must be one of %s (got %r)" % (MATH_MODES, mode))
    _math_mode = mode
    bump_epoch()


def get_math_mode():
    return _math_mode


def math_flag():
    return MATH_F32 if _math_mode == "f32" else (MATH_F16X2 if _math_mode == "f16x2" else 0)


def f16x2():
    return _math_mode == "f16x2"


_amax_pool, _amax_pos, _epoch = None, 0, 0
_wgen, _wlog = 0, {}
_WLOG_MAX = 64


def bump_epoch():
    global _epoch
    _epoch += 1
    _wlog.clear()


def amax_slot(device):
    global _amax_pool, _amax_pos
    if _amax_pool is None or _amax_pos >= _amax_pool.numel() or _amax_pool.device != device:
        _amax_pool, _amax_pos = torch.zeros(4096, dtype=torch.float32, device=device), 0
    s = _amax_pool[_amax_pos:_amax_pos + 1]
    _amax_pos += 1
    return s


def _extent(t):
    st = t.untyped_storage()
    key, lo = st.data_ptr(), t.data_ptr()
    span = 1
    for n, s in zip(t.shape, t.stride()):
        if n == 0:
            return key, lo, lo, False
        span += (n - 1) * s
    hi = lo + span * t.element_size()
    return key, lo, hi, lo <= key and hi >= key + st.nbytes()


def _note_write(t):
    global _wgen
    _wgen += 1
    key, lo, hi, whole = _extent(t)
    if whole:
        _wlog[key] = [_wgen, []]
    else:
        log = _wlog.setdefault(key, [0, []])
        log[1].append((_wgen, lo, hi))
        if len(log[1]) > _WLOG_MAX:
            log[0] = log[1].pop(0)[0]
    return key, lo, hi


def set_amax(t, slot, _ext=None):
    key, lo, hi = _ext if _ext is not None else _extent(t)[:3]
    t._lvt_amax = (slot, t._version, _epoch, t.data_ptr(), key, _wgen, lo, hi)
    return t


def drop_amax(t):
    t._lvt_amax = None
    _note_write(t)


AMAX_CHECK = bool(os.environ.get("LVT_AMAX_CHECK"))


def _checked(slot, t):
    if AMAX_CHECK and not torch.cuda.is_current_stream_capturing():
        have, real = float(slot), float(t.detach().abs().max()) if t.numel() else 0.0
        if not have >= real:
            raise LvtError("stale max |.| record: %g recorded, %g in the tensor of shape %s (an in-place kernel wrapper that "
                           "did not call binding.drop_amax?)" % (have, real, tuple(t.shape)))
    return slot


def _valid_amax(t):
    rec = getattr(t, "_lvt_amax", None)
    if rec is None or rec[1] != t._version or rec[2] != _epoch or rec[3] != t.data_ptr():
        return None
    log = _wlog.get(rec[4])
    if log is not None:
        gen = rec[5]
        if gen < log[0]:
            return None
        for g, lo, hi in reversed(log[1]):
            if g <= gen:
                break
            if lo < rec[7] and rec[6] < hi:
                return None
    return rec[0]


def new_amax(t):
    ext = _note_write(t)
    slot = amax_slot(t.device)
    set_amax(t, slot, ext)
    return slot


def amax_of(t):
    slot = _valid_amax(t)
    if slot is not None:
        return _checked(slot, t)
    base = t._base
    if base is not None:
        slot = _valid_amax(base)
        if slot is not None:
            return _checked(slot, t)
    src = t
    if not t.is_contiguous():
        if base is None or not base.is_contiguous():
            raise LvtError("amax_of: non-contiguous tensor without a contiguous base")
        src = base
    require(src)
    slot = amax_slot(src.device)
    check(lib().lvt_amax(ptr(src), src.numel(), ptr(slot), stream_ptr()), "lvt_amax")
    AMAX_FALLBACKS[0] += 1
    if AMAX_TRACE is not None:
        import traceback
        fr = [f for f in traceback.extract_stack()[:-1] if "binding.py" not in f.filename][-3:]
        key = " < ".join("%s:%d" % (os.path.basename(f.filename), f.lineno) for f in reversed(fr)) + " %s" % (tuple(src.shape),)
        AMAX_TRACE[key] = AMAX_TRACE.get(key, 0) + 1
    set_amax(src, slot)
    return slot


def out_amax(t):
    if _math_mode == "f16x2":
        return ptr(new_amax(t))
    drop_amax(t)
    return None


def amax_prefetch(tensors):
    if _math_mode != "f16x2":
        return
    todo = [t for t in tensors if t is not None and t.is_cuda and _valid_amax(t) is None and t.is_contiguous() and t.numel() > 0]
    if not todo:
        return
    arr = (AmaxEntry * len(todo))()
    for e, t in zip(arr, todo):
        slot = amax_slot(t.device)
        e.x, e.n, e.out = t.data_ptr(), t.numel(), slot.data_ptr()
        set_amax(t, slot)
    check(lib().lvt_amax_multi(arr, len(todo), stream_ptr()), "lvt_amax_multi")


def prefetch_module_weights(module):
    if _math_mode != "f16x2":
        return
    plan = module.__dict__.get("_lvt_prefetch_plan")
    if plan is None:
        plan = []
        for m in module.modules():
            packed = getattr(m, "packed_qkv", None)
            skip = ("w_q", "w_k", "w_v") if packed is not None else ()
            names = [name for name, p in m.named_parameters(recurse=False)
                     if name not in skip and (p.dim() >= 2 or isinstance(m, torch.nn.LayerNorm))]
            if packed is not None or names:
                plan.append((m, packed is not None, names))
        module.__dict__["_lvt_prefetch_plan"] = plan
    todo = []
    for m, has_packed, names in plan:
        if has_packed:
            todo.append(m.packed_qkv())
        params = m._parameters
        for name in names:
            todo.append(params[name])
    amax_prefetch(todo)


def amax_merged(*tensors):
    slots = [amax_of(t) for t in tensors]
    out = amax_slot(tensors[0].device)
    for i in range(0, len(slots), 2):
        check(lib().lvt_amax_merge(ptr(slots[i]), ptr(slots[i + 1]) if i + 1 < len(slots) else None, ptr(out), stream_ptr()),
              "lvt_amax_merge")
    return out


AMAX_TRACE = {} if os.environ.get("LVT_AMAX_TRACE") else None
AMAX_FALLBACKS = [0]


def amax_io(a=None, b=None, c=None):
    if _math_mode != "f16x2":
        if c is not None:
            drop_amax(c)
        return None
    io = AmaxIO()
    io.a = amax_of(a).data_ptr() if a is not None else None
    io.b = amax_of(b).data_ptr() if b is not None else None
    io.c = new_amax(c).data_ptr() if c is not None else None
    return io


def io_ref(io):
    return C.byref(io) if io is not None else None


def declared_symbols():
    return sorted(lib()._lvt_sigs.keys())


def require(*tensors):
    for t in tensors:
        if t is None:
            continue
        if not t.is_cuda:
            raise LvtError("lvt_amd kernels need tensors on a MI355X (got device %s); there is no CPU "
                           "fallback" % t.device)
        if not t.is_contiguous():
            raise LvtError("lvt_amd kernels need contiguous tensors")


def check(rc, what=""):
    if rc != 0:
        raise LvtError("%s failed (rc=%d): %s" % (what, rc, lib().lvt_last_error().decode()))


_raw_stream = getattr(torch._C, "_cuda_getCurrentRawStream", None)


def stream_ptr():
    if _raw_stream is not None:
        return C.c_void_p(_raw_stream(torch.cuda.current_device()))
    return C.c_void_p(torch.cuda.current_stream().cuda_stream)


def ptr(t):
    return C.c_void_p(t.data_ptr()) if t is not None else C.c_void_p(0)


class KernelTimer:

    def __init__(self):
        self.records = []

    def begin(self):
        ev = torch.cuda.Event(enable_timing=True)
        ev.record()
        return ev

    def end(self, key, flops, start):
        ev = torch.cuda.Event(enable_timing=True)
        ev.record()
        self.records.append((key, flops, start, ev))

    def summary(self):
        torch.cuda.synchronize()
        out = {}
        for key, flops, a, b in self.records:
            d = out.setdefault(key, {"launches": 0, "ms": 0.0, "flops": 0.0})
            d["launches"] += 1
            d["ms"] += a.elapsed_time(b)
            d["flops"] += flops
        return out


TIMER = None
RELU_TRACE = None


_ws = {}


def workspace(nbytes, device, tag="default"):
    if torch.cuda.is_current_stream_capturing():
        raise LvtError("binding.workspace(%r) requested during hipGraph capture: captured launches must use scratch "
                       "owned by the object that owns the graph" % (tag,))
    key = (device, tag, torch.cuda.current_stream(device).cuda_stream)
    buf = _ws.get(key)
    if buf is None or buf.numel() < nbytes:
        buf = torch.empty(max(int(nbytes), 1 << 20), dtype=torch.uint8, device=device)
        _ws[key] = buf
    return buf
```

lvt_amd/hip/convnet.py:

```python

import torch

from . import binding as L
from . import gemm as G
from . import ew
from . import norm as BN

class Layer:

    def __init__(self, kind, kernel, stride, pad, cin, cout, act="", res_from=-1, norm=""):
        self.kind, self.kernel, self.stride, self.pad = kind, kernel, stride, pad
        self.cin, self.cout, self.act, self.res_from = cin, cout, act, res_from
        self.norm = norm
        self.resamples = kind in ("pool", "up", "shuffle")

    @staticmethod
    def pad4(c):
        return (c + 3) // 4 * 4

    @classmethod
    def resample(cls, kind, channels):
        assert kind in ("pool", "up")
        return cls(kind, None, None, None, channels, channels)

    @classmethod
    def shuffle(cls, channels, act=""):
        assert act in ("", "relu", "tanh", "sigmoid")
        return cls("shuffle", None, None, None, 4 * channels, channels, act=act)

    def resampled_shape(self, shape):
        N, T, H, W, Cp = shape
        if self.kind == "pool":
            return (N, T, H // 2, W // 2, Cp)
        return (N, T, 2 * H, 2 * W, Cp if self.kind == "up" else Layer.pad4(self.cout))


def _geom(layer, x_shape):
    N, T, H, W, _ = x_shape
    ci, co = Layer.pad4(layer.cin), Layer.pad4(layer.cout)
    if layer.kind == "conv":
        return G.conv_geom(N, T, H, W, ci, co, layer.kernel, layer.stride, layer.pad)
    To, Ho, Wo = [(i - 1) * s - 2 * p + k for i, s, p, k in zip((T, H, W), layer.stride, layer.pad, layer.kernel)]
    g = G.conv_geom(N, To, Ho, Wo, co, ci, layer.kernel, layer.stride, layer.pad)
    assert (g.To, g.Ho, g.Wo) == (T, H, W), "ConvTranspose geometry mismatch"
    return g


def _padded_bias(layer, b):
    co = Layer.pad4(layer.cout)
    if b is None or b.numel() == co:
        return b
    return torch.cat([b, b.new_zeros(co - b.numel())])


def _act_flag(ly):
    if ly.act == "sigmoid":
        return L.EPI_SIGMOID | L.epi_pad(Layer.pad4(ly.cout) - ly.cout)
    return {"": 0, "relu": L.EPI_RELU, "leaky": L.EPI_LEAKY, "tanh": L.EPI_TANH}[ly.act]


def _world():
    dist = torch.distributed
    return dist.get_world_size() if dist.is_available() and dist.is_initialized() else 1


def _batch_stats(ly, nm):
    return ly.norm in ("bn", "syncbn") and nm.training


def _running_affine(ly, nm):
    co = Layer.pad4(ly.cout)
    return BN.finalize(ly.cout, co, nm.weight, nm.bias, nm.running_mean, nm.running_var, eps=nm.eps, flags=L.BN_RUNNING)


def _normalise(ly, nm, y, res):
    co = Layer.pad4(ly.cout)
    if _batch_stats(ly, nm):
        if nm.momentum is None:
            raise L.LvtError("BatchNorm momentum=None (cumulative average) is not implemented")
        st = BN.stats(y)
        nranks = _world() if ly.norm == "syncbn" else 1
        if nranks > 1:
            allst = torch.zeros(nranks, 2, co, dtype=torch.float32, device=y.device)
            allst[torch.distributed.get_rank()].copy_(st)
            torch.distributed.all_reduce(allst)
            st, flags = allst, L.BN_UPDATE
        else:
            flags = L.BN_UPDATE | L.BN_UNBIASED | L.BN_COUNT
        scale, shift, saved = BN.finalize(ly.cout, co, nm.weight, nm.bias, nm.running_mean, nm.running_var, stats=st,
                                          nranks=nranks, count=y.numel() // co, num_batches_tracked=nm.num_batches_tracked,
                                          momentum=nm.momentum, eps=nm.eps, flags=flags)
        batch = True
    else:
        scale, shift, saved = _running_affine(ly, nm)
        nranks, batch = 1, False
    out = BN.apply(y, scale, shift, res=res, act=_act_flag(ly))
    return out, (scale, saved, batch, nranks)


def stack_forward(layers, x, params, want_grad=True, norms=None):
    outs, geoms, packed = [], [], []
    norms = norms if norms is not None else [None] * len(layers)
    if not want_grad and all(nm is None or not _batch_stats(ly, nm) for ly, nm in zip(layers, norms)):
        todo = [i for i, nm in enumerate(norms) if nm is not None]
        if todo:
            params = list(params)
            folded = BN.fold([(params[i][0].detach(), layers[i].kind == "convT", norms[i], Layer.pad4(layers[i].cout))
                              for i in todo])
            for i, wb in zip(todo, folded):
                params[i] = wb
        norms = [None] * len(layers)
    pb = G.PackBatch()
    shape = tuple(x.shape)
    for i, (ly, (w, b)) in enumerate(zip(layers, params)):
        if ly.resamples:
            shape = ly.resampled_shape(shape)
            geoms.append(None)
            packed.append(None)
            continue
        g = _geom(ly, shape)
        wt = wph = wq = None
        if ly.kind == "conv":
            wp = pb.plain(g, w, ly.cin, ly.cout)
            if want_grad and i > 0 and G.bwd_data_by_phases(g):
                wph = pb.phases(g, w, ly.cin, ly.cout)
            if G.fwd_by_parity(g):
                wq = pb.parity(g, w, ly.cin, ly.cout)
            if want_grad and G.bwd_data_as_conv(g):
                wt = pb.t(g, w, ly.cin, ly.cout)
            shape = (g.N, g.To, g.Ho, g.Wo, g.Co)
        else:
            wp = pb.plain(g, w, ly.cout, ly.cin)
            if G.bwd_data_by_phases(g):
                wph = pb.phases(g, w, ly.cout, ly.cin)
            if want_grad and G.fwd_by_parity(g):
                wq = pb.parity(g, w, ly.cout, ly.cin)
            shape = (g.N, g.Ti, g.Hi, g.Wi, g.Ci)
        geoms.append(g)
        packed.append((wp, wt, wph, wq))
    pb.launch()
    cur = x
    pre, bn_saved = [None] * len(layers), [None] * len(layers)
    for i, (ly, (w, b)) in enumerate(zip(layers, params)):
        if ly.resamples:
            if ly.kind == "shuffle":
                cur = ew.pixel_shuffle2(cur, ly.cout, ly.act)
            else:
                cur = ew.pool2x2(cur) if ly.kind == "pool" else ew.upsample2x2(cur)
            outs.append(cur)
            continue
        g, (wp, wt, wph, wq) = geoms[i], packed[i]
        nm = norms[i]
        seen = (g.N, g.Ti, g.Hi, g.Wi) if ly.kind == "conv" else (g.N, g.To, g.Ho, g.Wo)
        assert seen == tuple(cur.shape[:4]), "geometry of the pre-pass does not match the activation"
        res = outs[ly.res_from] if ly.res_from >= 0 else None
        if nm is not None:
            if ly.kind == "conv":
                y = G.conv_fwd(g, cur, wp, wq=wq)
            else:
                y = G.conv_bwd_data(g, cur, wp, wph=wph)
            pre[i] = y
            y, bn_saved[i] = _normalise(ly, nm, y, res)
            outs.append(y)
            cur = y
            continue
        bias = _padded_bias(ly, b)
        if ly.kind == "conv":
            y = G.conv_fwd(g, cur, wp, bias=bias, res=res, flags=_act_flag(ly), wq=wq)
        elif (ly.cout <= 3 and ly.kernel == (1, 4, 4) and ly.stride == (1, 2, 2) and ly.pad == (0, 1, 1)
              and ly.cin % 16 == 0 and res is None and ly.act in ("", "tanh", "sigmoid")):
            y = G.convT4_fwd(cur, w, b, _act_flag(ly) & (L.EPI_TANH | L.EPI_SIGMOID))
        else:
            y = G.conv_bwd_data(g, cur, wp, bias=bias, res=res, flags=_act_flag(ly), wph=wph)
        outs.append(y)
        cur = y
    return outs, (geoms, packed, norms, pre, bn_saved)


def _bn_backward(ly, nm, gp, y, bn_saved):
    scale, saved, batch, nranks = bn_saved
    co = Layer.pad4(ly.cout)
    if ly.norm == "frozen":
        return BN.bwd_apply(gp, None, scale, train=False), None
    sums = BN.bwd_reduce(gp, y, saved)
    dg = (sums[1, :ly.cout].clone(), sums[0, :ly.cout].clone())
    if not batch:
        return BN.bwd_apply(gp, None, scale, train=False), dg
    if nranks > 1:
        sums = sums.clone()
        torch.distributed.all_reduce(sums)
    return BN.bwd_apply(gp, y, scale, saved, sums, n=nranks * (y.numel() // co), train=True), dg


def stack_backward(layers, x, outs, saved, grad_out, need_input_grad=False):
    geoms, packed, norms, pre, bn_saved = saved
    n = len(layers)
    last = layers[-1]
    if last.act == "tanh":
        gpre = ew.tanh_bwd(grad_out, outs[-1])
    elif last.act == "sigmoid":
        gpre = ew.sigmoid_bwd(grad_out, outs[-1])
    elif last.act in ("relu", "leaky"):
        raise L.LvtError("a ReLU-terminated stack is not used by the reference architectures")
    else:
        gpre = grad_out
    res_user = {ly.res_from: i for i, ly in enumerate(layers) if ly.res_from >= 0}
    gpres = [None] * n
    gpres[n - 1] = gpre
    grads = [None] * n
    norm_grads = [None] * n
    gx = None
    for i in range(n - 1, -1, -1):
        ly = layers[i]
        if ly.resamples:
            grads[i] = (None, None)
            if i == 0 and not need_input_grad:
                break
            prev = layers[i - 1] if i > 0 else None
            if ly.kind == "shuffle":
                if (i - 1) in res_user or (prev is not None and prev.act):
                    raise L.LvtError("a pixel shuffle must follow a convolution without activation that is no residual source")
                gin = ew.pixel_unshuffle2(gpres[i], ly.cout)
                if i > 0:
                    gpres[i - 1] = gin
                else:
                    gx = gin
                continue
            if (i - 1) in res_user or (prev is not None and prev.act in ("tanh", "sigmoid")):
                raise L.LvtError("a pool / upsample layer follows conv + (Leaky)ReLU layers only")
            mask = outs[i - 1] if (prev is not None and prev.act in ("relu", "leaky")) else None
            leaky = prev is not None and prev.act == "leaky"
            if ly.kind == "pool":
                gin = ew.upsample2x2(gpres[i], 0.25, mask=mask, leaky=leaky)
            else:
                gin = ew.pool2x2(gpres[i], 1.0, mask=mask, leaky=leaky)
            if i > 0:
                gpres[i - 1] = gin
            else:
                gx = gin
            continue
        g, (wp, wt, wph, wq) = geoms[i], packed[i]
        inp = outs[i - 1] if i > 0 else x
        gp = gpres[i]
        if norms[i] is not None:
            gp, norm_grads[i] = _bn_backward(ly, norms[i], gp, pre[i], bn_saved[i])
        co = Layer.pad4(ly.cout)
        db = None
        if norms[i] is not None:
            if ly.kind == "conv":
                dw = G.conv_bwd_weight(g, inp, gp, ly.cin, ly.cout)
            else:
                dw = G.conv_bwd_weight(g, gp, inp, ly.cout, ly.cin)
        elif ly.kind == "conv":
            dw, db = G.conv_bwd_weight(g, inp, gp, ly.cin, ly.cout, want_bias=True)
        else:
            dw, db = G.conv_bwd_weight(g, gp, inp, ly.cout, ly.cin, want_bias=True, bias_of_x=True)
        if norms[i] is None and db is None:
            db = G.colsum(gp, gp.numel() // co, co)[:ly.cout]
        grads[i] = (dw, db)
        if i == 0 and not need_input_grad:
            break
        prev = layers[i - 1] if i > 0 else None
        res = gpres[res_user[i - 1]] if (i - 1) in res_user else None
        mask = outs[i - 1] if (prev is not None and prev.act in ("relu", "leaky")) else None
        lk = L.EPI_LEAKY_MASK if (prev is not None and prev.act == "leaky") else 0
        if prev is not None and prev.act in ("tanh", "sigmoid"):
            raise L.LvtError("%s is only supported on the last layer of a stack" % prev.act)
        if ly.kind == "conv":
            gin = G.conv_bwd_data(g, gp, wp, res=res, mask=mask, flags=lk, wt=wt, wph=wph)
        else:
            gin = G.conv_fwd(g, gp, wp, res=res, mask=mask, flags=lk, wq=wq)
        if i > 0:
            gpres[i - 1] = gin
        else:
            gx = gin
    return gx, grads, [d for d in norm_grads if d is not None]
```

lvt_amd/hip/ew.py:

```python
import ctypes as C

import torch

from . import binding as L


def _f32(*shape, like):
    return torch.empty(*shape, dtype=torch.float32, device=like.device)


def to_channels_last(x_bcr, ldo, mode=0, a=None, s=None):
    L.require(x_bcr, a, s)
    B, Cc, R = x_bcr.shape
    out = _f32(B, R, ldo, like=x_bcr)
    L.check(L.lib().lvt_to_channels_last(L.ptr(x_bcr), B, Cc, R, ldo, mode, L.ptr(a), L.ptr(s), L.ptr(out),
                                         L.out_amax(out), L.stream_ptr()), "lvt_to_channels_last")
    return out


def to_channels_first(x_brc, Cc, mode=0, a=None, s=None, lo=0.0, hi=0.0):
    L.require(x_brc, a, s)
    B, R, ldi = x_brc.shape
    out = _f32(B, Cc, R, like=x_brc)
    L.check(L.lib().lvt_to_channels_first(L.ptr(x_brc), B, Cc, R, ldi, mode, L.ptr(a), L.ptr(s), lo, hi,
                                          L.ptr(out), L.stream_ptr()), "lvt_to_channels_first")
    return out


def _red_ws(dev):
    n = L.lib().lvt_reduce_workspace_bytes()
    return L.workspace(n, dev, "reduce"), n


def mse_fwd(a, b, denom, scale=1.0, l1=False):
    L.require(a, b)
    out = _f32(1, like=a)
    ws, n = _red_ws(a.device)
    L.check((L.lib().lvt_l1_fwd if l1 else L.lib().lvt_mse_fwd)(L.ptr(a), L.ptr(b), a.numel(), float(denom), scale, L.ptr(out), L.ptr(ws), n,
                                L.stream_ptr()), "lvt_mse_fwd")
    return out.view(())


def mse_bwd(a, b, denom, scale=1.0, gout=None, add=None, tanh_of_a=False, l1=False):
    L.require(a, b, gout, add)
    out = torch.empty_like(a)
    L.check((L.lib().lvt_l1_bwd if l1 else L.lib().lvt_mse_bwd)(L.ptr(a), L.ptr(b), a.numel(), float(denom), scale, L.ptr(gout), L.ptr(add),
                                1 if tanh_of_a else 0, L.ptr(out), L.out_amax(out), L.stream_ptr()), "lvt_mse_bwd")
    return out


def tanh_bwd(g, y):
    L.require(g, y)
    out = torch.empty_like(g)
    L.check(L.lib().lvt_tanh_bwd(L.ptr(g), L.ptr(y), g.numel(), L.ptr(out), L.out_amax(out), L.stream_ptr()), "lvt_tanh_bwd")
    return out


def sigmoid_bwd(g, y):
    L.require(g, y)
    out = torch.empty_like(g)
    L.check(L.lib().lvt_sigmoid_bwd(L.ptr(g), L.ptr(y), g.numel(), L.ptr(out), L.out_amax(out), L.stream_ptr()), "lvt_sigmoid_bwd")
    return out


def mask_flags(mask, leaky):
    if mask is None:
        return 0
    return L.EPI_MASK | (L.EPI_LEAKY_MASK if leaky else 0)


def _resample(fn, name, x, out_hw, scale, mask, leaky):
    L.require(x, mask)
    N, H, W, Cp = x.shape[0], x.shape[-3], x.shape[-2], x.shape[-1]
    if x.numel() != N * H * W * Cp:
        raise L.LvtError("%s: frames only (N, 1, H, W, C) or (N, H, W, C), got %s" % (name, tuple(x.shape)))
    out = torch.empty(tuple(x.shape[:-3]) + out_hw + (Cp,), dtype=torch.float32, device=x.device)
    if mask is not None and tuple(mask.shape) != tuple(out.shape):
        raise L.LvtError("%s: the mask must have the output's shape %s, got %s" % (name, tuple(out.shape), tuple(mask.shape)))
    L.check(fn(L.ptr(x), N, H, W, Cp, float(scale), L.ptr(mask), mask_flags(mask, leaky), L.ptr(out), L.out_amax(out),
               L.stream_ptr()), name)
    return out


def pool2x2(x, scale=0.25, mask=None, leaky=False):
    return _resample(L.lib().lvt_pool2x2, "lvt_pool2x2", x, (x.shape[-3] // 2, x.shape[-2] // 2), scale, mask, leaky)


def upsample2x2(x, scale=1.0, mask=None, leaky=False):
    return _resample(L.lib().lvt_upsample2x2, "lvt_upsample2x2", x, (2 * x.shape[-3], 2 * x.shape[-2]), scale, mask, leaky)


_SHUFFLE_ACTS = {"": 0, "relu": L.EPI_RELU, "tanh": L.EPI_TANH, "sigmoid": L.EPI_SIGMOID}


def _frames(name, x):
    if x.dim() in (4, 5):
        N, H, W, Cx = x.shape[0], x.shape[-3], x.shape[-2], x.shape[-1]
        if x.numel() == N * H * W * Cx:
            return N, H, W, Cx
    raise L.LvtError("%s: frames only (N, 1, H, W, C) or (N, H, W, C), got %s" % (name, tuple(x.shape)))


def pixel_shuffle2(x, C, act=""):
    L.require(x)
    N, H, W, Cx = _frames("lvt_pixel_shuffle2", x)
    if C <= 0 or Cx != 4 * C:
        raise L.LvtError("lvt_pixel_shuffle2: %d channels in, 4 * C = %d expected" % (Cx, 4 * C))
    if isinstance(act, str):
        if act not in _SHUFFLE_ACTS:
            raise L.LvtError("lvt_pixel_shuffle2: act %r is none of %s" % (act, sorted(_SHUFFLE_ACTS)))
        flag = _SHUFFLE_ACTS[act]
    else:
        flag = act & ~L.epi_pad(3)
    out = torch.empty(tuple(x.shape[:-3]) + (2 * H, 2 * W, (C + 3) // 4 * 4), dtype=torch.float32, device=x.device)
    L.check(L.lib().lvt_pixel_shuffle2(L.ptr(x), N, H, W, C, flag, L.ptr(out), L.out_amax(out), L.stream_ptr()), "lvt_pixel_shuffle2")
    return out


def pixel_unshuffle2(g, C):
    L.require(g)
    N, H2, W2, Cp = _frames("lvt_pixel_unshuffle2", g)
    if C <= 0 or Cp != (C + 3) // 4 * 4 or H2 % 2 or W2 % 2:
        raise L.LvtError("lvt_pixel_unshuffle2: (.., %d, %d, %d) is not the shuffle of C = %d channels" % (H2, W2, Cp, C))
    out = torch.empty(tuple(g.shape[:-3]) + (H2 // 2, W2 // 2, 4 * C), dtype=torch.float32, device=g.device)
    L.check(L.lib().lvt_pixel_unshuffle2(L.ptr(g), N, H2 // 2, W2 // 2, C, L.ptr(out), L.out_amax(out), L.stream_ptr()),
            "lvt_pixel_unshuffle2")
    return out


def axpy(x, alpha=1.0, alpha_dev=None, add=None):
    L.require(x, alpha_dev, add)
    out = torch.empty_like(x)
    L.check(L.lib().lvt_axpy(L.ptr(x), L.ptr(add), x.numel(), L.ptr(alpha_dev), alpha, L.ptr(out), L.stream_ptr()),
            "lvt_axpy")
    return out


def add_periodic_(x, table, P):
    L.require(x, table)
    d = x.shape[-1]
    L.check(L.lib().lvt_add_periodic(L.ptr(x), L.ptr(table), x.numel() // d, P, d, L.stream_ptr()),
            "lvt_add_periodic")
    L.drop_amax(x)
    return x


def layernorm_fwd(x, w, b, eps=1e-5, save_stats=True):
    L.require(x, w, b)
    d = x.shape[-1]
    rows = x.numel() // d
    y = torch.empty_like(x)
    mean = _f32(rows, like=x) if save_stats else None
    rstd = _f32(rows, like=x) if save_stats else None
    f16 = L.f16x2()
    L.check(L.lib().lvt_layernorm_fwd(L.ptr(x), rows, d, eps, L.ptr(w), L.ptr(b), L.ptr(y), L.ptr(mean),
                                      L.ptr(rstd), L.out_amax(y), L.ptr(L.amax_of(w)) if f16 else None,
                                      L.ptr(L.amax_of(b)) if f16 else None, L.stream_ptr()), "lvt_layernorm_fwd")
    return y, mean, rstd


def layernorm_fwd_p2(x, w, b, eps=1e-5):
    L.require(x, w, b)
    d = x.shape[-1]
    rows = x.numel() // d
    y = torch.empty_like(x)
    yp = torch.empty_like(x)
    mean, rstd = _f32(rows, like=x), _f32(rows, like=x)
    L.check(L.lib().lvt_layernorm_fwd_p2(L.ptr(x), rows, d, eps, L.ptr(w), L.ptr(b), L.ptr(y), L.ptr(yp), L.ptr(mean),
                                         L.ptr(rstd), L.out_amax(y), L.ptr(L.amax_of(w)), L.ptr(L.amax_of(b)),
                                         L.stream_ptr()), "lvt_layernorm_fwd_p2")
    return y, yp, mean, rstd


def layernorm_bwd(dy, x, mean, rstd, w, add=None):
    L.require(dy, x, mean, rstd, w, add)
    d = x.shape[-1]
    rows = x.numel() // d
    dx = torch.empty_like(x)
    dw, db = _f32(d, like=x), _f32(d, like=x)
    n = L.lib().lvt_layernorm_bwd_workspace_bytes(d)
    ws = L.workspace(n, x.device, "ln")
    L.check(L.lib().lvt_layernorm_bwd(L.ptr(dy), L.ptr(x), L.ptr(mean), L.ptr(rstd), L.ptr(w), rows, d, L.ptr(add),
                                      L.ptr(dx), L.ptr(dw), L.ptr(db), L.out_amax(dx), L.ptr(ws), n, L.stream_ptr()),
            "lvt_layernorm_bwd")
    return dx, dw, db


def row_gather(x, perm, S):
    L.require(x, perm)
    d = x.shape[-1]
    out = torch.empty_like(x)
    L.check(L.lib().lvt_row_gather(L.ptr(x), L.ptr(perm), x.numel() // (S * d), S, d, L.ptr(out), L.stream_ptr()),
            "lvt_row_gather")
    if L.f16x2() and L._valid_amax(x) is not None:
        L.set_amax(out, L._valid_amax(x))
    return out
```

lvt_amd/hip/vq.py:

```python
import os

import torch

from . import binding as L


VQ_COARSE = 1 << 17
VQ_GENERIC = 1 << 22
_COARSE_DEFAULT = bool(os.environ.get("LVT_VQ_COARSE"))


def nearest(z, codebooks, P, coarse=None, generic=False):
    L.require(z, codebooks)
    rows, ldz = z.shape
    num, K, D = codebooks.shape
    idx = torch.empty(rows // P, num, P, dtype=torch.int64, device=z.device)
    lib = L.lib()
    nws = max(lib.lvt_vq_nearest_workspace_bytes(rows, num, K), lib.lvt_vq_nearest_generic_workspace_bytes(num, D, K))
    ws = L.workspace(nws, z.device, "vq_nearest")
    flags = L.math_flag() | (VQ_COARSE if (coarse if coarse is not None else _COARSE_DEFAULT) else 0) | (VQ_GENERIC if generic else 0)
    L.check(lib.lvt_vq_nearest(L.ptr(z), rows, ldz, num, D, K, L.ptr(codebooks), L.ptr(idx), P, flags,
                               L.ptr(ws), nws, L.stream_ptr()), "lvt_vq_nearest")
    return idx


def nearest_single(z, weight, chunk_rows=1 << 16):
    from . import gemm as G
    L.require(z, weight)
    rows, D = z.shape
    K = weight.shape[0]
    idx = torch.empty(rows, dtype=torch.int64, device=z.device)
    w = weight.detach()
    scores = torch.empty(min(rows, chunk_rows), K, dtype=torch.float32, device=z.device)
    for r0 in range(0, rows, chunk_rows):
        r1 = min(rows, r0 + chunk_rows)
        G.gemm(z[r0:r1], w, scores, r1 - r0, K, D)
        L.check(L.lib().lvt_vq_argmax_scores(L.ptr(scores), r1 - r0, K, K, L.ptr(w), D, L.ptr(idx[r0:r1]), L.stream_ptr()),
                "lvt_vq_argmax_scores")
    return idx


def gather(idx, codebooks):
    L.require(idx, codebooks)
    n, num, P = idx.shape
    _, K, D = codebooks.shape
    out = torch.empty(n * P, num * D, dtype=torch.float32, device=idx.device)
    L.check(L.lib().lvt_vq_gather(L.ptr(idx), L.ptr(codebooks), n * P, num, D, K, P, L.ptr(out), num * D,
                                  L.stream_ptr()), "lvt_vq_gather")
    if L.f16x2():
        L.set_amax(out, L.amax_of(codebooks))
    return out


def ema_accumulate(idx, z, K, out=None):
    L.require(idx, z)
    n, num, P = idx.shape
    rows, ldz = z.shape
    D = ldz // num
    if out is None:
        stats = torch.empty(num, K, D + 1, dtype=torch.float32, device=z.device)
    else:
        L.require(out)
        if out.shape != (num, K, D + 1) or out.dtype != torch.float32 or out.device != z.device:
            raise L.LvtError("ema_accumulate: out must be a float32 (%d, %d, %d) tensor on %s" % (num, K, D + 1, z.device))
        stats = out
    lib = L.lib()
    nws = lib.lvt_vq_ema_workspace_bytes(rows, num, D, K)
    ws = L.workspace(nws, z.device, "ema")
    L.check(lib.lvt_vq_ema_accumulate(L.ptr(idx), L.ptr(z), rows, ldz, num, D, K, P, L.ptr(stats), L.ptr(ws), nws,
                                      L.stream_ptr()), "lvt_vq_ema_accumulate")
    return stats


def ema_finalize(stats, running_size, running_sum, weight, decay=0.99, eps=1e-5):
    L.require(stats, running_size, running_sum, weight)
    num, K, D = weight.shape
    L.check(L.lib().lvt_vq_ema_finalize(L.ptr(stats), num, D, K, decay, eps, L.ptr(running_size),
                                        L.ptr(running_sum), L.ptr(weight), L.stream_ptr()), "lvt_vq_ema_finalize")
    L.drop_amax(weight)


_M64 = (1 << 64) - 1


def _mix64(z):
    z = ((z ^ (z >> 30)) * 0xBF58476D1CE4E5B9) & _M64
    z = ((z ^ (z >> 27)) * 0x94D049BB133111EB) & _M64
    return z ^ (z >> 31)


def restart_row(seed, pass_, i, k, R, K):
    h = _mix64((seed ^ (pass_ * 0x9E3779B97F4A7C15) ^ (i << 32 | k)) & _M64)
    lo, hi = k * R // K, (k + 1) * R // K
    return lo + (h % (hi - lo) if hi > lo else 0)


def restart_buffer(num, K, D, device):
    ns = num * K * (D + 1)
    flat = torch.empty(ns + num * K * D, dtype=torch.float32, device=device)
    return flat, flat[:ns].view(num, K, D + 1), flat[ns:].view(num, K, D)


def restart_candidates(z, cand, P, rank, world, seed, pass_counter, shared_index=False):
    L.require(z, cand, pass_counter)
    rows, ldz = z.shape
    num, K, D = cand.shape
    L.check(L.lib().lvt_vq_restart_candidates(L.ptr(z), rows, ldz, num, D, K, P, rank, world, seed, L.ptr(pass_counter),
                                              int(bool(shared_index)), L.ptr(cand), L.stream_ptr()),
            "lvt_vq_restart_candidates")


def ema_finalize_restart(stats, cand, running_size, running_sum, weight, threshold, health, restarts_total, pass_counter,
                         decay=0.99, eps=1e-5):
    L.require(stats, cand, running_size, running_sum, weight, health, restarts_total, pass_counter)
    num, K, D = weight.shape
    L.check(L.lib().lvt_vq_ema_finalize_restart(L.ptr(stats), L.ptr(cand), num, D, K, decay, eps, threshold,
                                                L.ptr(running_size), L.ptr(running_sum), L.ptr(weight), L.ptr(health),
                                                L.ptr(restarts_total), L.ptr(pass_counter), L.stream_ptr()),
            "lvt_vq_ema_finalize_restart")
    L.drop_amax(weight)
```

lvt_amd/modeling/convstack.py:

```python
import torch
from torch import nn

from ..hip import binding as L
from ..hip import convnet, ew


class _ConvStackFn(torch.autograd.Function):

    @staticmethod
    def forward(ctx, x, layers, layers_grad, norms, *flat):
        params = [(flat[2 * i], flat[2 * i + 1]) for i in range(len(layers))]
        with torch.no_grad():
            outs, saved = convnet.stack_forward(layers, x, params, want_grad=layers_grad and any(ctx.needs_input_grad),
                                                norms=norms)
        ctx.layers, ctx.saved, ctx.outs, ctx.x = layers, saved, outs, x
        ctx.shapes = [tuple(p.shape) if p is not None else None for p in flat]
        return outs[-1]

    @staticmethod
    def backward(ctx, gy):
        gy = gy.contiguous()
        with torch.no_grad():
            gx, grads, norm_grads = convnet.stack_backward(ctx.layers, ctx.x, ctx.outs, ctx.saved, gy,
                                                           need_input_grad=ctx.needs_input_grad[0])
        flat = []
        for i, (dw, db) in enumerate(grads):
            flat.append(dw.view(ctx.shapes[2 * i]) if dw is not None else None)
            flat.append(db.contiguous().view(ctx.shapes[2 * i + 1]) if db is not None else None)
        for dgamma, dbeta in norm_grads:
            flat += [dgamma, dbeta]
        ctx.outs = ctx.saved = None
        return (gx, None, None, None) + tuple(flat)


def run_stack(x_cl, layers, params, norms=None):
    flat = [t for wb in params for t in wb]
    if norms is not None:
        flat += [t for ly, m in zip(layers, norms) if ly.norm in ("bn", "syncbn") for t in (m.weight, m.bias)]
    return _ConvStackFn.apply(x_cl, layers, torch.is_grad_enabled(), norms, *flat)


def nchw_to_cl(x, cpad=None):
    L.require(x)
    n, c, h, w = x.shape
    cp = cpad or (c + 3) // 4 * 4
    return ew.to_channels_last(x.reshape(n, c, h * w), cp).view(n, 1, h, w, cp)


def cl_to_nchw(y, c):
    n, _, h, w, cp = y.shape
    return ew.to_channels_first(y.view(n, h * w, cp), c).view(n, c, h, w)


class _LayoutIn(torch.autograd.Function):
    @staticmethod
    def forward(ctx, x):
        ctx.c = x.shape[1]
        return nchw_to_cl(x.contiguous())

    @staticmethod
    def backward(ctx, g):
        return cl_to_nchw(g.contiguous(), ctx.c)


class _LayoutOut(torch.autograd.Function):
    @staticmethod
    def forward(ctx, y, c):
        ctx.cp = y.shape[-1]
        return cl_to_nchw(y, c)

    @staticmethod
    def backward(ctx, g):
        return nchw_to_cl(g.contiguous(), ctx.cp), None


SUPPORTED_NORMS = ("", "BN", "SyncBN", "FrozenBN")
_OUT_ACTIVATIONS = {"": None, "sigmoid": nn.Sigmoid, "tanh": nn.Tanh}


def out_activation_module(name):
    if name not in _OUT_ACTIVATIONS:
        raise ValueError("Unknown activation %r" % (name,))
    cls = _OUT_ACTIVATIONS[name]
    return cls() if cls is not None else None


def act_after(nxt):
    if isinstance(nxt, (nn.ReLU, ResBlock)):
        return "relu"
    if isinstance(nxt, nn.LeakyReLU):
        if nxt.negative_slope != 0.2:
            raise NotImplementedError("LeakyReLU slope %r: the kernels implement 0.2 only" % (nxt.negative_slope,))
        return "leaky"
    if isinstance(nxt, nn.Tanh):
        return "tanh"
    if isinstance(nxt, nn.Sigmoid):
        return "sigmoid"
    return ""


def check_norm(norm, spectral):
    if (norm or "") not in SUPPORTED_NORMS or spectral:
        raise NotImplementedError("lvt_amd implements NORM in {%s} without spectral norm for ResEncoder / ResDecoder; got "
                                  "norm=%r spectral=%r" % (", ".join(repr(n) for n in SUPPORTED_NORMS), norm, spectral))


class NaiveSyncBatchNorm(nn.BatchNorm2d):

    def __init__(self, *args, stats_mode="", **kwargs):
        super().__init__(*args, **kwargs)
        if stats_mode != "":
            raise NotImplementedError("NaiveSyncBatchNorm: only stats_mode '' is implemented")
        self._stats_mode = stats_mode


class FrozenBatchNorm2d(nn.Module):

    _version = 3

    def __init__(self, num_features, eps=1e-5):
        super().__init__()
        self.num_features, self.eps = num_features, eps
        identity = {"weight": torch.ones(num_features), "bias": torch.zeros(num_features),
                    "running_mean": torch.zeros(num_features), "running_var": torch.ones(num_features) - eps}
        for name, t in identity.items():
            self.register_buffer(name, t)

    def _load_from_state_dict(self, state_dict, prefix, local_metadata, *args):
        saved = local_metadata.get("version")
        old = saved is None or saved < 2
        for name in ("running_mean", "running_var"):
            if old and prefix + name not in state_dict:
                state_dict[prefix + name] = torch.zeros_like(self.running_mean) if name == "running_mean" \
                    else torch.ones_like(self.running_var)
        if saved is not None and saved < 3:
            state_dict[prefix + "running_var"] = state_dict[prefix + "running_var"] - self.eps
        super()._load_from_state_dict(state_dict, prefix, local_metadata, *args)

    def extra_repr(self):
        return "%d, eps=%g" % (self.num_features, self.eps)


_NORM_MODULES = {"BN": nn.BatchNorm2d, "SyncBN": NaiveSyncBatchNorm, "FrozenBN": FrozenBatchNorm2d}


def norm_layer(layer, norm):
    if norm:
        layer.bias = None
        layer = nn.Sequential(layer, _NORM_MODULES[norm](layer.out_channels))
    return layer


def split_norm(m):
    if isinstance(m, nn.Sequential):
        conv, nm = m[0], m[1]
        kind = "frozen" if isinstance(nm, FrozenBatchNorm2d) else "syncbn" if isinstance(nm, NaiveSyncBatchNorm) else "bn"
        return conv, nm, kind
    return m, None, ""


def is_conv(m, cls):
    return isinstance(m, cls) or (isinstance(m, nn.Sequential) and len(m) == 2 and isinstance(m[0], cls))


def plain_plan(layers):
    Layer = convnet.Layer
    mods = list(layers)
    plan, owners, norms = [], [], []
    for i, m in enumerate(mods):
        nxt = mods[i + 1] if i + 1 < len(mods) else None
        if is_conv(m, nn.Conv2d):
            conv, nm, kind = split_norm(m)
            k, s, p = conv.kernel_size[0], conv.stride[0], conv.padding[0]
            plan.append(Layer("conv", (1, k, k), (1, s, s), (0, p, p), conv.in_channels, conv.out_channels,
                              act=act_after(nxt), norm=kind))
            owners.append(conv)
            norms.append(nm)
        elif isinstance(m, (nn.AvgPool2d, nn.Upsample)):
            if isinstance(m, nn.AvgPool2d):
                ok, kind = m.kernel_size == 2 and m.stride == 2 and m.padding == 0, "pool"
            else:
                ok, kind = m.scale_factor == 2 and m.mode == "nearest" and m.size is None, "up"
            if not ok or not plan:
                raise NotImplementedError("only AvgPool2d(2) / nearest Upsample(scale_factor=2) behind a convolution: %r" % (m,))
            plan.append(Layer.resample(kind, plan[-1].cout))
            owners.append(None)
            norms.append(None)
        elif not isinstance(m, (nn.LeakyReLU, nn.ReLU, nn.Tanh, nn.Sigmoid)):
            raise NotImplementedError("no plan for %r" % (m,))
    return plan, owners, (norms if any(n is not None for n in norms) else None)


def plan_params(owners):
    return [(m.weight, m.bias) if m is not None else (None, None) for m in owners]


class ResBlock(nn.Module):

    def __init__(self, dim, dim_res, norm="BN"):
        super().__init__()
        check_norm(norm, False)
        self.block = nn.Sequential(nn.ReLU(True), norm_layer(nn.Conv2d(dim, dim_res, 3, 1, 1), norm), nn.ReLU(True),
                                   norm_layer(nn.Conv2d(dim_res, dim, 1), norm))


class _TokensIn(torch.autograd.Function):

    @staticmethod
    def forward(ctx, x):
        ctx.shape = tuple(x.shape)
        B, C = x.shape[:2]
        R = x[0, 0].numel()
        return ew.to_channels_last(x.contiguous().view(B, C, R), C).view(B * R, C)

    @staticmethod
    def backward(ctx, g):
        B, C = ctx.shape[:2]
        R = g.shape[0] // B
        return ew.to_channels_first(g.contiguous().view(B, R, C), C).view(ctx.shape)


class _TokensOut(torch.autograd.Function):

    @staticmethod
    def forward(ctx, tok, B, C, T, H, W):
        return ew.to_channels_first(tok.contiguous().view(B, T * H * W, tok.shape[-1]), C).view(B, C, T, H, W)

    @staticmethod
    def backward(ctx, g):
        B, C = g.shape[:2]
        R = g[0, 0].numel()
        return ew.to_channels_last(g.contiguous().view(B, C, R), C).view(B * R, C), None, None, None, None, None
```

lvt_amd/modeling/generator/convdecoder.py:

```python
from torch import nn

from .. import convstack
from .build import GENERATOR_REGISTRY
from .generator import Generator


@GENERATOR_REGISTRY.register()
class ConvDecoder(Generator):
    @classmethod
    def from_config(cls, cfg, **kwargs):
        g = cfg.MODEL.GENERATOR
        return cls(in_channels=g.IN_CHANNELS, nf=g.NF, out_channels=g.OUT_CHANNELS, norm=g.NORM,
                   use_spectral_norm=g.SPECTRAL, n_layers=g.N_LAYERS, out_activation=g.OUT_ACTIVATION)

    def __init__(self, in_channels, nf, out_channels, norm, use_spectral_norm, n_layers, out_activation):
        super().__init__()
        convstack.check_norm(norm, use_spectral_norm)
        out_act = convstack.out_activation_module(out_activation)
        norm = norm or ""

        def conv(ci, co, nm):
            return convstack.norm_layer(nn.Conv2d(ci, co, 3, stride=1, padding=1), nm)

        mods = []
        kp = in_channels
        for scale in range(n_layers - 1, -1, -1):
            k = nf << scale
            mods += [conv(kp, k, norm), nn.LeakyReLU(0.2, True), conv(k, k, norm), nn.LeakyReLU(0.2, True),
                     nn.Upsample(scale_factor=2)]
            kp = k
        if kp != nf:
            raise ValueError("ConvDecoder: the last convolution reads %d channels but the one in front writes NF = %d "
                             "(N_LAYERS 0 needs IN_CHANNELS == NF)" % (kp, nf))
        mods += [conv(kp, nf, ""), conv(kp, out_channels, "")]
        if out_act is not None:
            mods.append(out_act)
        self.layers = nn.Sequential(*mods)
        self.in_channels, self.out_channels = in_channels, out_channels
        self._plan, self._owners, self._norms = convstack.plain_plan(self.layers)

    def forward_cl(self, z_cl):
        return convstack.run_stack(z_cl, self._plan, convstack.plan_params(self._owners), self._norms)

    def forward(self, z):
        y = self.forward_cl(convstack._LayoutIn.apply(z))
        return convstack._LayoutOut.apply(y, self.out_channels)
```

lvt_amd/modeling/generator/resdecoder.py:

```python
from torch import nn

from ...hip.convnet import Layer
from .. import convstack
from .build import GENERATOR_REGISTRY
from .generator import Generator


class _ResTrunkDecoder(Generator):

    @classmethod
    def from_config(cls, cfg, **kwargs):
        g = cfg.MODEL.GENERATOR
        return cls(in_channels=g.IN_CHANNELS, nf=g.NF, res_channels=g.RES_CHANNELS, out_channels=g.OUT_CHANNELS,
                   norm=g.NORM, use_spectral_norm=g.SPECTRAL, n_layers=g.N_LAYERS,
                   out_activation=kwargs.get("out_activation", g.OUT_ACTIVATION), stride=kwargs.get("stride", 4))

    def __init__(self, in_channels, nf, res_channels, out_channels, norm, use_spectral_norm, n_layers,
                 out_activation, stride):
        super().__init__()
        convstack.check_norm(norm, use_spectral_norm)
        norm = norm or ""
        nl = convstack.norm_layer
        mods = [nl(nn.Conv2d(in_channels, nf, 3, 1, 1), norm)]
        mods += [convstack.ResBlock(nf, res_channels, norm) for _ in range(n_layers)]
        mods.append(nn.ReLU(True))
        mods += self._upscale(nf, out_channels, norm, stride)
        out_act = convstack.out_activation_module(out_activation)
        if out_act is not None:
            mods.append(out_act)
        self.layers = nn.Sequential(*mods)
        self.in_channels, self.out_channels = in_channels, out_channels
        self._plan = self._build_plan()

    def _build_plan(self):
        mods = list(self.layers)
        plan, owners, norms = [], [], []
        for i, m in enumerate(mods):
            nxt = mods[i + 1] if i + 1 < len(mods) else None
            act = convstack.act_after(nxt)
            if convstack.is_conv(m, nn.Conv2d) or convstack.is_conv(m, nn.ConvTranspose2d):
                m, nm, kind = convstack.split_norm(m)
                k, s, p = m.kernel_size[0], m.stride[0], m.padding[0]
                plan.append(Layer("convT" if isinstance(m, nn.ConvTranspose2d) else "conv", (1, k, k), (1, s, s), (0, p, p),
                                  m.in_channels, m.out_channels, act=act, norm=kind))
                owners.append(m)
                norms.append(nm)
            elif isinstance(m, convstack.ResBlock):
                (c3, n3, k3), (c1, n1, k1) = convstack.split_norm(m.block[1]), convstack.split_norm(m.block[3])
                src = len(plan) - 1
                plan.append(Layer("conv", (1, 3, 3), (1, 1, 1), (0, 1, 1), c3.in_channels, c3.out_channels, act="relu",
                                  norm=k3))
                owners.append(c3)
                norms.append(n3)
                plan.append(Layer("conv", (1, 1, 1), (1, 1, 1), (0, 0, 0), c1.in_channels, c1.out_channels, act=act,
                                  res_from=src, norm=k1))
                owners.append(c1)
                norms.append(n1)
            elif isinstance(m, nn.PixelShuffle):
                if m.upscale_factor != 2 or not plan or plan[-1].cout % 4:
                    raise NotImplementedError("only PixelShuffle(2) behind a convolution to 4 C channels: %r" % (m,))
                plan.append(Layer.shuffle(plan[-1].cout // 4, act=act))
                owners.append(None)
                norms.append(None)
        self._owners = owners
        self._norms = norms if any(n is not None for n in norms) else None
        return plan

    def forward_cl(self, z_cl):
        return convstack.run_stack(z_cl, self._plan, convstack.plan_params(self._owners), self._norms)

    def forward(self, z):
        y = self.forward_cl(convstack._LayoutIn.apply(z))
        return convstack._LayoutOut.apply(y, self.out_channels)


@GENERATOR_REGISTRY.register()
class ResDecoder(_ResTrunkDecoder):
    @staticmethod
    def _upscale(nf, out_channels, norm, stride):
        nl = convstack.norm_layer
        if stride == 4:
            return [nl(nn.ConvTranspose2d(nf, nf // 2, 4, 2, 1), norm), nn.ReLU(True),
                    nn.ConvTranspose2d(nf // 2, out_channels, 4, 2, 1)]
        if stride == 2:
            return [nl(nn.ConvTranspose2d(nf, out_channels, 4, 2, 1), norm)]
        raise ValueError


@GENERATOR_REGISTRY.register()
class ResShuffleDecoder(_ResTrunkDecoder):

    @staticmethod
    def _upscale(nf, out_channels, norm, stride):
        nl = convstack.norm_layer
        if stride == 4:
            return [nl(nn.Conv2d(nf, nf // 2 * 4, 3, 1, 1), norm), nn.PixelShuffle(2), nn.ReLU(True),
                    nn.Conv2d(nf // 2, out_channels * 4, 3, 1, 1), nn.PixelShuffle(2)]
        if stride == 2:
            return [nl(nn.Conv2d(nf, out_channels * 4, 3, 1, 1), norm), nn.PixelShuffle(2)]
        raise ValueError
```

lvt_amd/modeling/loss/loss.py:

```python
import torch
from torch import nn

from ...hip import ew


class _MseFn(torch.autograd.Function):

    @staticmethod
    def forward(ctx, a, b, denom, scale, l1=False):
        ctx.save_for_backward(a, b)
        ctx.denom, ctx.scale, ctx.l1 = denom, scale, l1
        return ew.mse_fwd(a, b, denom, scale, l1=l1)

    @staticmethod
    def backward(ctx, g):
        a, b = ctx.saved_tensors
        return ew.mse_bwd(a, b, ctx.denom, ctx.scale, gout=g.contiguous().view(1), l1=ctx.l1), None, None, None, None


def mse(a, b, denom=None, scale=1.0):
    return _MseFn.apply(a.contiguous(), b.contiguous(), float(denom if denom is not None else a.numel()), scale)


def l1(a, b, denom=None, scale=1.0):
    return _MseFn.apply(a.contiguous(), b.contiguous(), float(denom if denom is not None else a.numel()), scale, True)


class PixelLoss(nn.Module):
    def __init__(self, cfg):
        super().__init__()
        mode = cfg.LOSS.PIXEL.MODE
        if mode not in ("l1", "l2"):
            raise NotImplementedError
        self._fn = l1 if mode == "l1" else mse
        self._lambda = cfg.LOSS.PIXEL.LAMBDA

    def forward(self, input, target, denom=None):
        return self._fn(input, target, denom, self._lambda)
```

lvt_amd/modeling/meta_arch/vqvae.py:

```python
import os

from ...solver import build_lr_scheduler, build_optimizer
from ...utils.checkpoint import Checkpointer
from ..loss import PixelLoss
from ..loss.loss import mse
from ..vq import DVQEmbedding, SingleVQEmbedding
from .ae import AutoEncoderModel
from .build import META_ARCH_REGISTRY


@META_ARCH_REGISTRY.register()
class VQVAEModel(AutoEncoderModel):
    def __init__(self, cfg):
        super().__init__(cfg)
        cb = cfg.MODEL.CODEBOOK
        self.use_codebook_ema = cb.EMA
        if cb.NUM == 1:
            self.codebook = SingleVQEmbedding(cb.SIZE, cb.DIM, self.use_codebook_ema)
        else:
            self.codebook = DVQEmbedding(cb.NUM, cb.SIZE, cb.DIM, self.use_codebook_ema)
        if self.use_codebook_ema:
            self._set_requires_grad(self.codebook.parameters(), False)
        if cb.RESTART.ENABLED:
            self.codebook.enable_restart(cb.RESTART.THRESHOLD, max(cfg.SEED, 0))
        self.pixel_loss = PixelLoss(cfg)
        self.beta = cb.BETA
        self.to(self.device)

    def train(self, mode=True):
        super().train(mode)
        self.codebook.train(mode)
        return self

    def wrap_parallel(self, device_ids, broadcast_buffers):
        import torch
        import torch.distributed as dist
        from ...utils import comm
        super().wrap_parallel(device_ids, broadcast_buffers)
        if not self.use_codebook_ema:
            from ...engine.grad_reducer import BucketedGradReducer
            self._reducers.append(BucketedGradReducer(self.codebook.parameters()))
        if comm.get_world_size() > 1:
            with torch.no_grad():
                for t in self.codebook._flat():
                    if t is not None:
                        dist.broadcast(t, 0)

    def codebook_health(self):
        return self.codebook.health_scalars()

    def _generator_parameters(self):
        params = super()._generator_parameters()
        if not self.use_codebook_ema:
            params += list(self.codebook.parameters())
        return params

    def forward(self, data, mode="inference"):
        return super().forward(data, mode)

    def _latent_cl(self, x):
        return self.codebook.indices_cl(self.encoder.forward_cl(x))

    def _latent_public(self, latent):
        return latent

    def _decode_cl(self, latent):
        return self.generator.forward_cl(self.codebook.embed_cl(latent))

    def _supervised_loss_cl(self, x, return_x=False):
        z_e = self.encoder.forward_cl(x)
        z_q_st = self.codebook.straight_through_cl(z_e, defer=True)
        try:
            x_tilde = self.generator.forward_cl(z_q_st)
        except BaseException:
            self.codebook.abandon_ema()
            raise
        z_q_bar = self.codebook.finish_ema()
        c = len(self.cfg.MODEL.PIXEL_MEAN)
        loss = {
            "loss_reconstruction": self.pixel_loss(x_tilde, x, denom=x.numel() // x.shape[-1] * c),
            "loss_commitment": mse(z_e, z_q_bar.detach(), scale=self.beta),
        }
        if not self.use_codebook_ema:
            loss["loss_dict"] = mse(z_q_bar, z_e.detach())
        return (loss, x, x_tilde) if return_x else loss

    def _generator_loss_cl(self, x):
        return self._supervised_loss_cl(x)

    def compute_supervised_loss(self, x, return_x=False):
        return self._supervised_loss_cl(self._as_cl(x), return_x)

    def decode(self, latents):
        from .. import convstack
        self._require_gpu()
        y = self._decode_cl(latents.to(self.device))
        return convstack.cl_to_nchw(y, self.generator.out_channels)

    def configure_optimizers_and_checkpointers(self):
        o, c = super().configure_optimizers_and_checkpointers()
        if not self.use_codebook_ema:
            opt = build_optimizer(self.codebook, self.cfg, suffix="_G")
            o.append({"optimizer": opt, "scheduler": build_lr_scheduler(self.cfg, opt), "type": "generator"})
        os.makedirs(os.path.join(self.cfg.OUTPUT_DIR, "netC"), exist_ok=True)
        c.append({"checkpointer": Checkpointer(self.codebook, os.path.join(self.cfg.OUTPUT_DIR, "netC")),
                  "pretrained": self.cfg.MODEL.CODEBOOK.WEIGHTS})
        return o, c
```

lvt_amd/modeling/vq/vq_embedding.py:

```python
import torch
from torch import nn

from ...hip import binding as L
from ...hip import ew, vq
from ...layers.all_reduce import all_reduce_sum_async_
from ...utils import comm
from .. import convstack

SUPPORTED_GEOMETRY = ("sub-vector width DIM / NUM: a multiple of 16 from 16 to 256 (product quantiser, DVQEmbedding) or "
                      "DIM a multiple of 64 (one wide codebook, SingleVQEmbedding); codebook size SIZE: a multiple of 64 "
                      "from 64 to 2048")


def check_geometry(num, K, D, single=False):
    if num < 1 or D % num:
        raise NotImplementedError("CODEBOOK.DIM (%d) must be a multiple of CODEBOOK.NUM (%d); supported: %s"
                                  % (D, num, SUPPORTED_GEOMETRY))
    dg = D // num
    if single:
        ok_d = D % 64 == 0 and D > 0
    else:
        ok_d = dg % 16 == 0 and 16 <= dg <= 256
    if not ok_d:
        raise NotImplementedError("unsupported codebook geometry NUM=%d DIM=%d (sub-vector width %d); supported: %s"
                                  % (num, D, dg, SUPPORTED_GEOMETRY))
    if K % 64 or not 64 <= K <= 2048:
        raise NotImplementedError("unsupported codebook SIZE=%d; supported: %s" % (K, SUPPORTED_GEOMETRY))


class _RestartMixin:

    _restart = None

    def enable_restart(self, threshold=1.0, seed=0):
        threshold = float(threshold)
        if not self.ema:
            raise ValueError("codebook restart needs CODEBOOK.EMA: a trained codebook has no running_size")
        if not (0.0 <= threshold < float("inf")):
            raise ValueError("codebook restart: THRESHOLD must be finite and >= 0 (got %r)" % (threshold,))
        ngroups = getattr(self, "groups", self.num)
        dev = self._flat()[0].device
        self.register_buffer("restart_pass", torch.zeros(1, dtype=torch.int64, device=dev), persistent=False)
        self.register_buffer("restart_health", torch.zeros(ngroups, 3, device=dev), persistent=False)
        self.register_buffer("restart_total", torch.zeros(ngroups, dtype=torch.int64, device=dev), persistent=False)
        self._restart = (threshold, max(int(seed), 0))

    @property
    def restart_enabled(self):
        return self._restart is not None

    def _restart_now(self):
        return self._restart is not None and self.training

    def _accumulate(self, idx, z2d, P, shared_index):
        if not self._restart_now():
            stats = vq.ema_accumulate(idx, z2d, self.K)
            return stats, all_reduce_sum_async_(stats), None
        num = idx.shape[1]
        flat, stats, cand = vq.restart_buffer(num, self.K, z2d.shape[1] // num, z2d.device)
        vq.ema_accumulate(idx, z2d, self.K, out=stats)
        vq.restart_candidates(z2d, cand, P, comm.get_rank(), comm.get_world_size(), self._restart[1], self.restart_pass,
                              shared_index=shared_index)
        return stats, all_reduce_sum_async_(flat), cand

    def _finalize(self, stats, cand, rsize, rsum, w):
        if cand is None:
            vq.ema_finalize(stats, rsize, rsum, w, self.decay, self.eps)
        else:
            vq.ema_finalize_restart(stats, cand, rsize, rsum, w, self._restart[0], self.restart_health, self.restart_total,
                                    self.restart_pass, self.decay, self.eps)

    def health_scalars(self):
        if self._restart is None:
            return None
        n = self.num
        h = self.restart_health[:n].double()
        return h[:, 0].mean(), h[:, 1].sum(), self.restart_total[:n].sum().double()


class VQEmbedding(nn.Module):

    def __init__(self, K, D, ema):
        super().__init__()
        self.embedding = nn.Embedding(K, D)
        self.embedding.weight.data.uniform_(-1.0 / K, 1.0 / K)
        self.K, self.D, self.ema = K, D, ema
        if ema:
            self.eps, self.decay = 1e-5, 0.99
            self.register_buffer("running_size", torch.zeros(K))
            self.register_buffer("running_sum", self.embedding.weight.detach().clone())


class _StraightThroughFn(torch.autograd.Function):

    @staticmethod
    def forward(ctx, z2d, owner, P):
        w, rsize, rsum = owner._flat()
        idx = vq.nearest(z2d, w, P)
        z_q_st = vq.gather(idx, w)
        stats = work = None
        cand = None
        if owner.ema:
            stats, work, cand = owner._accumulate(idx, z2d, P, False)
        owner._pending = (idx, stats, work, cand)
        ctx.mark_non_differentiable(idx)
        return z_q_st, idx

    @staticmethod
    def backward(ctx, g_st, g_idx):
        return g_st, None, None


class _GatherWithGradFn(torch.autograd.Function):

    @staticmethod
    def forward(ctx, idx, owner, *weights):
        ctx.save_for_backward(idx)
        ctx.K, ctx.num, ctx.d = owner.K, owner.num, owner.D // owner.num
        return vq.gather(idx, owner._flat()[0])

    @staticmethod
    def backward(ctx, g):
        (idx,) = ctx.saved_tensors
        stats = vq.ema_accumulate(idx, g.contiguous(), ctx.K)
        return (None, None) + tuple(stats[i, :, :ctx.d].contiguous() for i in range(ctx.num))


class _SingleStraightThroughFn(torch.autograd.Function):

    @staticmethod
    def forward(ctx, z2d, owner, P):
        w = owner.embedding.weight.detach()
        idx = vq.nearest_single(z2d, w)
        idx_g = owner._group_idx(idx, P)
        z_q_st = vq.gather(idx_g, owner._grouped(w))
        stats = work = None
        cand = None
        if owner.ema:
            stats, work, cand = owner._accumulate(idx_g, z2d, P, True)
        owner._pending = (idx, idx_g, stats, work, cand)
        ctx.mark_non_differentiable(idx)
        return z_q_st, idx

    @staticmethod
    def backward(ctx, g_st, g_idx):
        return g_st, None, None


class _SingleGatherWithGradFn(torch.autograd.Function):

    @staticmethod
    def forward(ctx, idx_g, owner, weight):
        ctx.save_for_backward(idx_g)
        ctx.owner = owner
        return vq.gather(idx_g, owner._grouped(weight.detach()))

    @staticmethod
    def backward(ctx, g):
        (idx_g,) = ctx.saved_tensors
        o = ctx.owner
        stats = vq.ema_accumulate(idx_g, g.contiguous(), o.K)
        return None, None, stats[:, :, :64].permute(1, 0, 2).reshape(o.K, o.D).contiguous()


class SingleVQEmbedding(_RestartMixin, VQEmbedding):

    def __init__(self, K, D, ema):
        check_geometry(1, K, D, single=True)
        super().__init__(K, D, ema)
        self.num, self.groups = 1, D // 64
        self._pending = None

    def _grouped(self, t):
        if t.dim() == 1:
            return t.unsqueeze(0).expand(self.groups, self.K).contiguous()
        out = t.view(self.K, self.groups, 64).permute(1, 0, 2).contiguous()
        if L.f16x2() and L._valid_amax(t) is not None:
            L.set_amax(out, L._valid_amax(t))
        return out

    def _ungrouped(self, t):
        return t.permute(1, 0, 2).reshape(self.K, self.D)

    def _group_idx(self, idx, P):
        return idx.view(-1, 1, P).expand(-1, self.groups, P).contiguous()

    def _flat(self):
        return (self.embedding.weight.data, getattr(self, "running_size", None), getattr(self, "running_sum", None))

    def indices_cl(self, z_cl):
        n, _, h, w, d = z_cl.shape
        L.require(z_cl)
        return vq.nearest_single(z_cl.view(n * h * w, d), self.embedding.weight).view(n, h, w)

    def straight_through_cl(self, z_cl, defer=False):
        n, _, h, w, d = z_cl.shape
        L.require(z_cl)
        if self._pending is not None:
            raise L.LvtError("SingleVQEmbedding: the EMA update of the previous pass was never finished (finish_ema)")
        z_q_st, idx = _SingleStraightThroughFn.apply(z_cl.view(n * h * w, d), self, h * w)
        self.last_indices = idx.view(n, h, w)
        self._pending_shape = (n, 1, h, w, d)
        z_q_st = z_q_st.view(n, 1, h, w, d)
        return z_q_st if defer else (z_q_st, self.finish_ema())

    def finish_ema(self):
        if self._pending is None:
            raise L.LvtError("SingleVQEmbedding.finish_ema without a pending straight_through_cl")
        idx, idx_g, stats, work, cand = self._pending
        self._pending = None
        w = self.embedding.weight
        if stats is not None:
            if work is not None:
                work.wait()
            wg, rs, rsum = self._grouped(w.data), self._grouped(self.running_size), self._grouped(self.running_sum)
            self._finalize(stats, cand, rs, rsum, wg)
            with torch.no_grad():
                w.data.copy_(self._ungrouped(wg))
                self.running_size.copy_(rs[0])
                self.running_sum.copy_(self._ungrouped(rsum))
            L.drop_amax(w)
            return vq.gather(idx_g, wg).view(*self._pending_shape)
        return _SingleGatherWithGradFn.apply(idx_g, self, w).view(*self._pending_shape)

    def abandon_ema(self):
        pend, self._pending = self._pending, None
        if pend is not None and pend[3] is not None:
            pend[3].wait()

    def embed_cl(self, latents):
        n, h, w = latents.shape
        L.require(latents)
        out = vq.gather(self._group_idx(latents.contiguous().view(-1), h * w), self._grouped(self.embedding.weight.detach()))
        return out.view(n, 1, h, w, self.D)

    def forward(self, z_e_x, mode=""):
        if mode == "":
            return self.indices_cl(convstack._LayoutIn.apply(z_e_x))
        if mode == "st":
            st, bar = self.straight_through_cl(convstack._LayoutIn.apply(z_e_x))
            return convstack._LayoutOut.apply(st, self.D), convstack._LayoutOut.apply(bar, self.D)
        if mode == "emb":
            return self.embed_cl(z_e_x).squeeze(1)
        raise ValueError


class DVQEmbedding(_RestartMixin, nn.Module):
    def __init__(self, num, K, D, ema):
        super().__init__()
        check_geometry(num, K, D)
        self.num, self.D, self.K, self.ema = num, D, K, ema
        self.decay, self.eps = 0.99, 1e-5
        self.ve = nn.ModuleList([VQEmbedding(K, D // num, ema) for _ in range(num)])
        self._flat_w = self._flat_rs = self._flat_rsum = None

    def _flat(self):
        w0 = self.ve[0].embedding.weight
        fw = self._flat_w
        ok = fw is not None and fw.device == w0.device and all(
            self.ve[i].embedding.weight.data_ptr() == fw[i].data_ptr()
            and (not self.ema or (self.ve[i].running_size.data_ptr() == self._flat_rs[i].data_ptr()
                                  and self.ve[i].running_sum.data_ptr() == self._flat_rsum[i].data_ptr()))
            for i in range(self.num))
        if not ok:
            with torch.no_grad():
                fw = torch.stack([v.embedding.weight.data for v in self.ve]).contiguous()
                frs = frsum = None
                if self.ema:
                    frs = torch.stack([v.running_size for v in self.ve]).contiguous()
                    frsum = torch.stack([v.running_sum for v in self.ve]).contiguous()
                for i, v in enumerate(self.ve):
                    v.embedding.weight.data = fw[i]
                    if self.ema:
                        v.running_size = frs[i]
                        v.running_sum = frsum[i]
            self._flat_w, self._flat_rs, self._flat_rsum = fw, frs, frsum
        return self._flat_w, self._flat_rs, self._flat_rsum

    def indices_cl(self, z_cl):
        n, _, h, w, d = z_cl.shape
        L.require(z_cl)
        idx = vq.nearest(z_cl.view(n * h * w, d), self._flat()[0], h * w)
        return idx.view(n, self.num, h, w)

    def straight_through_cl(self, z_cl, defer=False):
        n, _, h, w, d = z_cl.shape
        L.require(z_cl)
        if getattr(self, "_pending", None) is not None:
            raise L.LvtError("DVQEmbedding: the EMA update of the previous pass was never finished (finish_ema)")
        z_q_st, idx = _StraightThroughFn.apply(z_cl.view(n * h * w, d), self, h * w)
        self.last_indices = idx.view(n, self.num, h, w)
        self._pending_shape = (n, 1, h, w, d)
        z_q_st = z_q_st.view(n, 1, h, w, d)
        return z_q_st if defer else (z_q_st, self.finish_ema())

    def finish_ema(self):
        pend = getattr(self, "_pending", None)
        if pend is None:
            raise L.LvtError("DVQEmbedding.finish_ema without a pending straight_through_cl")
        idx, stats, work, cand = pend
        self._pending = None
        w, rsize, rsum = self._flat()
        if stats is not None:
            if work is not None:
                work.wait()
            self._finalize(stats, cand, rsize, rsum, w)
        if not self.ema:
            return _GatherWithGradFn.apply(idx, self, *[v.embedding.weight for v in self.ve]).view(*self._pending_shape)
        return vq.gather(idx, w).view(*self._pending_shape)

    def abandon_ema(self):
        pend = getattr(self, "_pending", None)
        if pend is not None:
            self._pending = None
            if pend[2] is not None:
                pend[2].wait()

    def embed_cl(self, latents):
        n, num, h, w = latents.shape
        L.require(latents)
        out = vq.gather(latents.contiguous().view(n, num, h * w), self._flat()[0])
        return out.view(n, 1, h, w, self.D)

    def forward(self, z_e_x, mode=""):
        if mode == "":
            assert z_e_x.dim() == 4
            return self.indices_cl(convstack._LayoutIn.apply(z_e_x))
        if mode == "st":
            assert z_e_x.dim() == 4
            st, bar = self.straight_through_cl(convstack._LayoutIn.apply(z_e_x))
            return convstack._LayoutOut.apply(st, self.D), convstack._LayoutOut.apply(bar, self.D)
        if mode == "emb":
            return self.embed_cl(z_e_x).squeeze(1)
        raise ValueError
```

Baseline: 1442.

## Fuse VQ commitment loss with codebook gather and pixel loss into decoder head backward

Adds commit_fwd/commit_bwd kernels that read the quantized code vectors straight from the codebook through the indices, so z_q_bar no longer has to be materialised for the commitment MSE. The commitment gradient is folded into the straight-through backward through a link object. The reconstruction loss gradient is fused into the decoder's final activation backward via a head argument, and mse_bwd gains a sigmoid path for this. The forward reduction loop is also unrolled four ways. The cost is more complex autograd bookkeeping (weakrefs, handles, stale-link fallbacks) and a risk of subtle gradient or ordering bugs.

Measured after the change: 1454 (median of 6 runs). No clear change (+0.8%).

```diff
diff --git a/include/lvt_hip.h b/include/lvt_hip.h
--- a/include/lvt_hip.h
+++ b/include/lvt_hip.h
@@ -183,11 +183,17 @@
 int lvt_mse_fwd(const float *a, const float *b, long long n, double denom, float scale, float *out,
                 void *workspace, size_t workspace_bytes, void *stream);
 int lvt_mse_bwd(const float *a, const float *b, long long n, double denom, float scale,
-                const float *gout_dev, const float *add, int tanh_of_a, float *out, float *out_amax, void *stream);
+                const float *gout_dev, const float *add, int act_of_a, float *out, float *out_amax, void *stream);
 int lvt_l1_fwd(const float *a, const float *b, long long n, double denom, float scale, float *out,
                void *workspace, size_t workspace_bytes, void *stream);
 int lvt_l1_bwd(const float *a, const float *b, long long n, double denom, float scale,
-               const float *gout_dev, const float *add, int tanh_of_a, float *out, float *out_amax, void *stream);
+               const float *gout_dev, const float *add, int act_of_a, float *out, float *out_amax, void *stream);
+int lvt_vq_commit_fwd(const float *z, const long long *idx, const float *codebooks, long long rows, int ldz, int num, int D,
+                      int KC, int P, double denom, float scale, float *out, void *workspace, size_t workspace_bytes,
+                      void *stream);
+int lvt_vq_commit_bwd(const float *z, const long long *idx, const float *codebooks, long long rows, int ldz, int num, int D,
+                      int KC, int P, double denom, float scale, const float *gout_dev, const float *add, float *out,
+                      float *out_amax, void *stream);
 int lvt_tanh_bwd(const float *g, const float *y, long long n, float *out, float *out_amax, void *stream);
 int lvt_sigmoid_bwd(const float *g, const float *y, long long n, float *out, float *out_amax, void *stream);
 int lvt_axpy(const float *x, const float *add, long long n, const float *alpha_dev, float alpha,
diff --git a/lvt_amd/csrc/elementwise.hip b/lvt_amd/csrc/elementwise.hip
--- a/lvt_amd/csrc/elementwise.hip
+++ b/lvt_amd/csrc/elementwise.hip
@@ -71,19 +71,42 @@
 }
 
 #define RED_BLOCKS 1024
-template <int L1>
-__global__ void lvt_sqdiff_partial_kernel(const float *__restrict__ a, const float *__restrict__ b, long long n4,
-                                          float *__restrict__ partial) {
+struct DenseB {
+    const float *b;
+    __device__ __forceinline__ float4 operator()(long long i) const { return reinterpret_cast<const float4 *>(b)[i]; }
+};
+template <class I>
+struct CodeB {
+    const long long *idx; const float *cb;
+    int Q4, D4, num, KC, P;
+    __device__ __forceinline__ float4 operator()(long long i) const {
+        const I row = (I)i / (I)Q4;
+        const int c4 = (int)((I)i - row * (I)Q4);
+        const int g = c4 / D4, q = c4 - g * D4;
+        const I n = row / (I)P;
+        const long long k = idx[((long long)n * num + g) * P + (long long)(row - n * (I)P)];
+        return *reinterpret_cast<const float4 *>(cb + (((long long)g * KC + k) * D4 + q) * 4);
+    }
+};
+template <int L1, class BS>
+__device__ __forceinline__ void sqdiff_partial_body(const float *__restrict__ a, const BS b, long long n4, float *__restrict__ partial) {
     __shared__ float red[256];
     float s = 0.f;
-    for (long long i = (long long)blockIdx.x * blockDim.x + threadIdx.x; i < n4;
-         i += (long long)gridDim.x * blockDim.x) {
-        const float4 x = reinterpret_cast<const float4 *>(a)[i];
-        const float4 y = reinterpret_cast<const float4 *>(b)[i];
+    const long long step = (long long)gridDim.x * blockDim.x;
+    long long i = (long long)blockIdx.x * blockDim.x + threadIdx.x;
+    auto term = [](const float4 x, const float4 y) {
         const float d0 = x.x - y.x, d1 = x.y - y.y, d2 = x.z - y.z, d3 = x.w - y.w;
-        if (L1) s += (fabsf(d0) + fabsf(d1)) + (fabsf(d2) + fabsf(d3));
-        else s += (d0 * d0 + d1 * d1) + (d2 * d2 + d3 * d3);
-    }
+        if (L1) return (fabsf(d0) + fabsf(d1)) + (fabsf(d2) + fabsf(d3));
+        return (d0 * d0 + d1 * d1) + (d2 * d2 + d3 * d3);
+    };
+    for (; i + 3 * step < n4; i += 4 * step) {
+        float4 x[4], y[4];
+#pragma unroll
+        for (int u = 0; u < 4; ++u) { x[u] = reinterpret_cast<const float4 *>(a)[i + u * step]; y[u] = b(i + u * step); }
+#pragma unroll
+        for (int u = 0; u < 4; ++u) s += term(x[u], y[u]);
+    }
+    for (; i < n4; i += step) s += term(reinterpret_cast<const float4 *>(a)[i], b(i));
     red[threadIdx.x] = s;
     __syncthreads();
     for (int k = 128; k > 0; k >>= 1) {
@@ -91,6 +114,15 @@
         __syncthreads();
     }
     if (threadIdx.x == 0) partial[blockIdx.x] = red[0];
+}
+template <int L1>
+__global__ void lvt_sqdiff_partial_kernel(const float *__restrict__ a, const float *__restrict__ b, long long n4,
+                                          float *__restrict__ partial) {
+    sqdiff_partial_body<L1>(a, DenseB{b}, n4, partial);
+}
+template <class I>
+__global__ void lvt_vq_commit_fwd_kernel(const float *__restrict__ z, const CodeB<I> b, long long n4, float *__restrict__ partial) {
+    sqdiff_partial_body<0>(z, b, n4, partial);
 }
 __global__ void lvt_scalar_finish_kernel(const float *__restrict__ partial, int n, float scale,
                                          const float *__restrict__ denom_dev, float *__restrict__ out) {
@@ -138,26 +170,29 @@
     return LVT_OK;
 }
 
-template <int L1>
-__global__ void lvt_mse_bwd_kernel(const float *__restrict__ a, const float *__restrict__ b, long long n4, float c,
-                                   const float *__restrict__ gout, const float *__restrict__ add, int tanh_of_a,
-                                   float *__restrict__ out, float *__restrict__ out_amax) {
+template <int L1, class BS>
+__device__ __forceinline__ void mse_bwd_body(const float *__restrict__ a, const BS b, long long n4, float c,
+                                             const float *__restrict__ gout, const float *__restrict__ add, int act_of_a,
+                                             float *__restrict__ out, float *__restrict__ out_amax) {
     __shared__ float amax_scratch[4];
     float am = 0.f;
     const float g = (gout ? gout[0] : 1.0f) * c;
     for (long long i = (long long)blockIdx.x * blockDim.x + threadIdx.x; i < n4;
          i += (long long)gridDim.x * blockDim.x) {
         const float4 x = reinterpret_cast<const float4 *>(a)[i];
-        const float4 y = reinterpret_cast<const float4 *>(b)[i];
+        const float4 y = b(i);
         float4 r = make_float4(x.x - y.x, x.y - y.y, x.z - y.z, x.w - y.w);
         if (L1) r = make_float4((float)((r.x > 0.f) - (r.x < 0.f)), (float)((r.y > 0.f) - (r.y < 0.f)), (float)((r.z > 0.f) - (r.z < 0.f)),
                                 (float)((r.w > 0.f) - (r.w < 0.f)));
         r.x *= g; r.y *= g; r.z *= g; r.w *= g;
-        if (tanh_of_a) {
+        if (act_of_a == 1) {
             r.x *= 1.f - x.x * x.x; r.y *= 1.f - x.y * x.y; r.z *= 1.f - x.z * x.z; r.w *= 1.f - x.w * x.w;
+        } else if (act_of_a == 2) {
+            r.x *= x.x * (1.f - x.x); r.y *= x.y * (1.f - x.y); r.z *= x.z * (1.f - x.z); r.w *= x.w * (1.f - x.w);
         }
         if (add) {
             const float4 z = reinterpret_cast<const float4 *>(add)[i];
+            asm volatile("" : "+v"(r.x), "+v"(r.y), "+v"(r.z), "+v"(r.w));
             r.x += z.x; r.y += z.y; r.z += z.z; r.w += z.w;
         }
         reinterpret_cast<float4 *>(out)[i] = r;
@@ -165,20 +200,79 @@
     }
     if (out_amax) lvt_block_amax_commit(am, out_amax, amax_scratch);
 }
+template <int L1>
+__global__ void lvt_mse_bwd_kernel(const float *__restrict__ a, const float *__restrict__ b, long long n4, float c,
+                                   const float *__restrict__ gout, const float *__restrict__ add, int act_of_a,
+                                   float *__restrict__ out, float *__restrict__ out_amax) {
+    mse_bwd_body<L1>(a, DenseB{b}, n4, c, gout, add, act_of_a, out, out_amax);
+}
+template <class I>
+__global__ void lvt_vq_commit_bwd_kernel(const float *__restrict__ z, const CodeB<I> b, long long n4, float c,
+                                         const float *__restrict__ gout, const float *__restrict__ add,
+                                         float *__restrict__ out, float *__restrict__ out_amax) {
+    mse_bwd_body<0>(z, b, n4, c, gout, add, 0, out, out_amax);
+}
 extern "C" int lvt_mse_bwd(const float *a, const float *b, long long n, double denom, float scale,
-                           const float *gout_dev, const float *add, int tanh_of_a, float *out, float *out_amax, void *stream) {
-    LVT_REQUIRE(a && b && out && n > 0 && n % 4 == 0 && denom > 0, "mse_bwd: bad args");
+                           const float *gout_dev, const float *add, int act_of_a, float *out, float *out_amax, void *stream) {
+    LVT_REQUIRE(a && b && out && n > 0 && n % 4 == 0 && denom > 0 && act_of_a >= 0 && act_of_a <= 2, "mse_bwd: bad args");
     hipLaunchKernelGGL(lvt_mse_bwd_kernel<0>, dim3(grid_for(n / 4, 256, out_amax ? 2048 : 8192)), dim3(256), 0, (hipStream_t)stream, a, b,
-                       n / 4, (float)(2.0 * (double)scale / denom), gout_dev, add, tanh_of_a, out, out_amax);
+                       n / 4, (float)(2.0 * (double)scale / denom), gout_dev, add, act_of_a, out, out_amax);
     LVT_CHECK_LAUNCH("lvt_mse_bwd_kernel");
     return LVT_OK;
 }
 extern "C" int lvt_l1_bwd(const float *a, const float *b, long long n, double denom, float scale,
-                          const float *gout_dev, const float *add, int tanh_of_a, float *out, float *out_amax, void *stream) {
-    LVT_REQUIRE(a && b && out && n > 0 && n % 4 == 0 && denom > 0, "l1_bwd: bad args");
+                          const float *gout_dev, const float *add, int act_of_a, float *out, float *out_amax, void *stream) {
+    LVT_REQUIRE(a && b && out && n > 0 && n % 4 == 0 && denom > 0 && act_of_a >= 0 && act_of_a <= 2, "l1_bwd: bad args");
     hipLaunchKernelGGL(lvt_mse_bwd_kernel<1>, dim3(grid_for(n / 4, 256, out_amax ? 2048 : 8192)), dim3(256), 0, (hipStream_t)stream, a, b,
-                       n / 4, (float)((double)scale / denom), gout_dev, add, tanh_of_a, out, out_amax);
+                       n / 4, (float)((double)scale / denom), gout_dev, add, act_of_a, out, out_amax);
     LVT_CHECK_LAUNCH("lvt_mse_bwd_kernel<l1>");
+    return LVT_OK;
+}
+
+template <class I>
+static CodeB<I> commit_src(const long long *idx, const float *codebooks, int num, int D, int KC, int P) {
+    return CodeB<I>{idx, codebooks, num * D / 4, D / 4, num, KC, P};
+}
+static bool commit_args_ok(const float *z, const long long *idx, const float *codebooks, long long rows, int ldz, int num, int D,
+                           int KC, int P) {
+    return z && idx && codebooks && rows > 0 && num > 0 && D > 0 && D % 4 == 0 && KC > 0 && P > 0 && rows % P == 0 &&
+           ldz == num * D && lvt_aligned16(z) && lvt_aligned16(codebooks);
+}
+extern "C" int lvt_vq_commit_fwd(const float *z, const long long *idx, const float *codebooks, long long rows, int ldz, int num,
+                                 int D, int KC, int P, double denom, float scale, float *out, void *workspace,
+                                 size_t workspace_bytes, void *stream) {
+    LVT_REQUIRE(commit_args_ok(z, idx, codebooks, rows, ldz, num, D, KC, P) && out && denom > 0, "vq_commit_fwd: bad args");
+    LVT_REQUIRE(workspace && workspace_bytes >= lvt_reduce_workspace_bytes(), "vq_commit_fwd: workspace");
+    hipStream_t s = (hipStream_t)stream;
+    const long long n4 = rows * (num * D / 4);
+    const int blocks = grid_for(n4, 256 * 4, RED_BLOCKS);
+    if (n4 <= 0x7fffffffLL)
+        hipLaunchKernelGGL(lvt_vq_commit_fwd_kernel<unsigned>, dim3(blocks), dim3(256), 0, s, z,
+                           commit_src<unsigned>(idx, codebooks, num, D, KC, P), n4, (float *)workspace);
+    else
+        hipLaunchKernelGGL(lvt_vq_commit_fwd_kernel<long long>, dim3(blocks), dim3(256), 0, s, z,
+                           commit_src<long long>(idx, codebooks, num, D, KC, P), n4, (float *)workspace);
+    LVT_CHECK_LAUNCH("lvt_vq_commit_fwd_kernel");
+    hipLaunchKernelGGL(lvt_scalar_finish_kernel, dim3(1), dim3(256), 0, s, (const float *)workspace, blocks,
+                       (float)((double)scale / denom), (const float *)nullptr, out);
+    LVT_CHECK_LAUNCH("lvt_scalar_finish_kernel");
+    return LVT_OK;
+}
+extern "C" int lvt_vq_commit_bwd(const float *z, const long long *idx, const float *codebooks, long long rows, int ldz, int num,
+                                 int D, int KC, int P, double denom, float scale, const float *gout_dev, const float *add,
+                                 float *out, float *out_amax, void *stream) {
+    LVT_REQUIRE(commit_args_ok(z, idx, codebooks, rows, ldz, num, D, KC, P) && out && denom > 0 && lvt_aligned16(out) &&
+                (!add || lvt_aligned16(add)), "vq_commit_bwd: bad args");
+    const long long n4 = rows * (num * D / 4);
+    const dim3 grid(grid_for(n4, 256, out_amax ? 2048 : 8192));
+    const float c = (float)(2.0 * (double)scale / denom);
+    if (n4 <= 0x7fffffffLL)
+        hipLaunchKernelGGL(lvt_vq_commit_bwd_kernel<unsigned>, grid, dim3(256), 0, (hipStream_t)stream, z,
+                           commit_src<unsigned>(idx, codebooks, num, D, KC, P), n4, c, gout_dev, add, out, out_amax);
+    else
+        hipLaunchKernelGGL(lvt_vq_commit_bwd_kernel<long long>, grid, dim3(256), 0, (hipStream_t)stream, z,
+                           commit_src<long long>(idx, codebooks, num, D, KC, P), n4, c, gout_dev, add, out, out_amax);
+    LVT_CHECK_LAUNCH("lvt_vq_commit_bwd_kernel");
     return LVT_OK;
 }
 
diff --git a/lvt_amd/hip/binding.py b/lvt_amd/hip/binding.py
--- a/lvt_amd/hip/binding.py
+++ b/lvt_amd/hip/binding.py
@@ -174,6 +174,8 @@
         "lvt_mse_bwd": (ci, [vp, vp, cll, C.c_double, cf, vp, vp, ci, vp, vp, vp]),
         "lvt_l1_fwd": (ci, [vp, vp, cll, C.c_double, cf, vp, vp, sz, vp]),
         "lvt_l1_bwd": (ci, [vp, vp, cll, C.c_double, cf, vp, vp, ci, vp, vp, vp]),
+        "lvt_vq_commit_fwd": (ci, [vp, vp, vp, cll, ci, ci, ci, ci, ci, C.c_double, cf, vp, vp, sz, vp]),
+        "lvt_vq_commit_bwd": (ci, [vp, vp, vp, cll, ci, ci, ci, ci, ci, C.c_double, cf, vp, vp, vp, vp, vp]),
         "lvt_tanh_bwd": (ci, [vp, vp, cll, vp, vp, vp]),
         "lvt_sigmoid_bwd": (ci, [vp, vp, cll, vp, vp, vp]),
         "lvt_axpy": (ci, [vp, vp, cll, vp, cf, vp, vp]),
diff --git a/lvt_amd/hip/convnet.py b/lvt_amd/hip/convnet.py
--- a/lvt_amd/hip/convnet.py
+++ b/lvt_amd/hip/convnet.py
@@ -192,18 +192,28 @@
     return BN.bwd_apply(gp, y, scale, saved, sums, n=nranks * (y.numel() // co), train=True), dg
 
 
-def stack_backward(layers, x, outs, saved, grad_out, need_input_grad=False):
+def _head_backward(act, grad_out, y):
+    if act == "tanh":
+        return ew.tanh_bwd(grad_out, y)
+    if act == "sigmoid":
+        return ew.sigmoid_bwd(grad_out, y)
+    if act in ("relu", "leaky"):
+        raise L.LvtError("a ReLU-terminated stack is not used by the reference architectures")
+    return grad_out
+
+
+def stack_backward(layers, x, outs, saved, grad_out, need_input_grad=False, head=None):
     geoms, packed, norms, pre, bn_saved = saved
     n = len(layers)
     last = layers[-1]
-    if last.act == "tanh":
-        gpre = ew.tanh_bwd(grad_out, outs[-1])
-    elif last.act == "sigmoid":
-        gpre = ew.sigmoid_bwd(grad_out, outs[-1])
-    elif last.act in ("relu", "leaky"):
-        raise L.LvtError("a ReLU-terminated stack is not used by the reference architectures")
+    if head is None:
+        gpre = _head_backward(last.act, grad_out, outs[-1])
     else:
-        gpre = grad_out
+        target, denom, scale, l1, gout = head
+        if last.act in ("relu", "leaky"):
+            raise L.LvtError("a ReLU-terminated stack is not used by the reference architectures")
+        other = _head_backward(last.act, grad_out, outs[-1]) if grad_out is not None else None
+        gpre = ew.mse_bwd(outs[-1], target, denom, scale, gout=gout, add=other, act_of_a=last.act, l1=l1)
     res_user = {ly.res_from: i for i, ly in enumerate(layers) if ly.res_from >= 0}
     gpres = [None] * n
     gpres[n - 1] = gpre
diff --git a/lvt_amd/hip/ew.py b/lvt_amd/hip/ew.py
--- a/lvt_amd/hip/ew.py
+++ b/lvt_amd/hip/ew.py
@@ -41,11 +41,15 @@
     return out.view(())
 
 
-def mse_bwd(a, b, denom, scale=1.0, gout=None, add=None, tanh_of_a=False, l1=False):
+_HEAD_ACTS = {"": 0, None: 0, "tanh": 1, "sigmoid": 2}
+
+
+def mse_bwd(a, b, denom, scale=1.0, gout=None, add=None, tanh_of_a=False, l1=False, act_of_a=""):
     L.require(a, b, gout, add)
     out = torch.empty_like(a)
+    act = 1 if tanh_of_a else _HEAD_ACTS[act_of_a]
     L.check((L.lib().lvt_l1_bwd if l1 else L.lib().lvt_mse_bwd)(L.ptr(a), L.ptr(b), a.numel(), float(denom), scale, L.ptr(gout), L.ptr(add),
-                                1 if tanh_of_a else 0, L.ptr(out), L.out_amax(out), L.stream_ptr()), "lvt_mse_bwd")
+                                act, L.ptr(out), L.out_amax(out), L.stream_ptr()), "lvt_mse_bwd")
     return out
 
 
diff --git a/lvt_amd/hip/vq.py b/lvt_amd/hip/vq.py
--- a/lvt_amd/hip/vq.py
+++ b/lvt_amd/hip/vq.py
@@ -49,6 +49,37 @@
                                   L.stream_ptr()), "lvt_vq_gather")
     if L.f16x2():
         L.set_amax(out, L.amax_of(codebooks))
+    return out
+
+
+def _commit_args(z, idx, codebooks):
+    L.require(z, idx, codebooks)
+    n, num, P = idx.shape
+    _, K, D = codebooks.shape
+    rows, ldz = z.shape
+    if rows != n * P or ldz != num * D or codebooks.shape[0] != num:
+        raise L.LvtError("vq commit: z %s, idx %s and codebooks %s do not belong together"
+                         % (tuple(z.shape), tuple(idx.shape), tuple(codebooks.shape)))
+    return rows, ldz, num, D, K, P
+
+
+def commit_fwd(z, idx, codebooks, denom, scale=1.0):
+    rows, ldz, num, D, K, P = _commit_args(z, idx, codebooks)
+    out = torch.empty(1, dtype=torch.float32, device=z.device)
+    lib = L.lib()
+    nws = lib.lvt_reduce_workspace_bytes()
+    ws = L.workspace(nws, z.device, "reduce")
+    L.check(lib.lvt_vq_commit_fwd(L.ptr(z), L.ptr(idx), L.ptr(codebooks), rows, ldz, num, D, K, P, float(denom), scale, L.ptr(out),
+                                  L.ptr(ws), nws, L.stream_ptr()), "lvt_vq_commit_fwd")
+    return out.view(())
+
+
+def commit_bwd(z, idx, codebooks, denom, scale=1.0, gout=None, add=None):
+    rows, ldz, num, D, K, P = _commit_args(z, idx, codebooks)
+    L.require(gout, add)
+    out = torch.empty_like(z)
+    L.check(L.lib().lvt_vq_commit_bwd(L.ptr(z), L.ptr(idx), L.ptr(codebooks), rows, ldz, num, D, K, P, float(denom), scale,
+                                      L.ptr(gout), L.ptr(add), L.ptr(out), L.out_amax(out), L.stream_ptr()), "lvt_vq_commit_bwd")
     return out
 
 
diff --git a/lvt_amd/modeling/convstack.py b/lvt_amd/modeling/convstack.py
--- a/lvt_amd/modeling/convstack.py
+++ b/lvt_amd/modeling/convstack.py
@@ -8,36 +8,45 @@
 class _ConvStackFn(torch.autograd.Function):
 
     @staticmethod
-    def forward(ctx, x, layers, layers_grad, norms, *flat):
+    def forward(ctx, x, layers, layers_grad, norms, head, *flat):
         params = [(flat[2 * i], flat[2 * i + 1]) for i in range(len(layers))]
         with torch.no_grad():
             outs, saved = convnet.stack_forward(layers, x, params, want_grad=layers_grad and any(ctx.needs_input_grad),
                                                 norms=norms)
-        ctx.layers, ctx.saved, ctx.outs, ctx.x = layers, saved, outs, x
+        ctx.layers, ctx.saved, ctx.outs, ctx.x, ctx.head = layers, saved, outs, x, head
         ctx.shapes = [tuple(p.shape) if p is not None else None for p in flat]
-        return outs[-1]
-
-    @staticmethod
-    def backward(ctx, gy):
-        gy = gy.contiguous()
+        if head is None:
+            return outs[-1]
+        ctx.set_materialize_grads(False)
+        target, denom, scale, l1 = head
+        return outs[-1], ew.mse_fwd(outs[-1], target, denom, scale, l1=l1)
+
+    @staticmethod
+    def backward(ctx, gy, gloss=None):
+        gy = gy.contiguous() if gy is not None else None
+        head = None
+        if ctx.head is not None and gloss is not None:
+            head = ctx.head + (gloss.contiguous().view(1),)
+        elif gy is None:
+            raise L.LvtError("conv stack backward without a gradient")
         with torch.no_grad():
             gx, grads, norm_grads = convnet.stack_backward(ctx.layers, ctx.x, ctx.outs, ctx.saved, gy,
-                                                           need_input_grad=ctx.needs_input_grad[0])
+                                                           need_input_grad=ctx.needs_input_grad[0], head=head)
         flat = []
         for i, (dw, db) in enumerate(grads):
             flat.append(dw.view(ctx.shapes[2 * i]) if dw is not None else None)
             flat.append(db.contiguous().view(ctx.shapes[2 * i + 1]) if db is not None else None)
         for dgamma, dbeta in norm_grads:
             flat += [dgamma, dbeta]
-        ctx.outs = ctx.saved = None
-        return (gx, None, None, None) + tuple(flat)
-
-
-def run_stack(x_cl, layers, params, norms=None):
+        ctx.outs = ctx.saved = ctx.head = None
+        return (gx, None, None, None, None) + tuple(flat)
+
+
+def run_stack(x_cl, layers, params, norms=None, head=None):
     flat = [t for wb in params for t in wb]
     if norms is not None:
         flat += [t for ly, m in zip(layers, norms) if ly.norm in ("bn", "syncbn") for t in (m.weight, m.bias)]
-    return _ConvStackFn.apply(x_cl, layers, torch.is_grad_enabled(), norms, *flat)
+    return _ConvStackFn.apply(x_cl, layers, torch.is_grad_enabled(), norms, head, *flat)
 
 
 def nchw_to_cl(x, cpad=None):
diff --git a/lvt_amd/modeling/generator/convdecoder.py b/lvt_amd/modeling/generator/convdecoder.py
--- a/lvt_amd/modeling/generator/convdecoder.py
+++ b/lvt_amd/modeling/generator/convdecoder.py
@@ -39,8 +39,8 @@
         self.in_channels, self.out_channels = in_channels, out_channels
         self._plan, self._owners, self._norms = convstack.plain_plan(self.layers)
 
-    def forward_cl(self, z_cl):
-        return convstack.run_stack(z_cl, self._plan, convstack.plan_params(self._owners), self._norms)
+    def forward_cl(self, z_cl, head=None):
+        return convstack.run_stack(z_cl, self._plan, convstack.plan_params(self._owners), self._norms, head=head)
 
     def forward(self, z):
         y = self.forward_cl(convstack._LayoutIn.apply(z))
diff --git a/lvt_amd/modeling/generator/resdecoder.py b/lvt_amd/modeling/generator/resdecoder.py
--- a/lvt_amd/modeling/generator/resdecoder.py
+++ b/lvt_amd/modeling/generator/resdecoder.py
@@ -66,8 +66,8 @@
         self._norms = norms if any(n is not None for n in norms) else None
         return plan
 
-    def forward_cl(self, z_cl):
-        return convstack.run_stack(z_cl, self._plan, convstack.plan_params(self._owners), self._norms)
+    def forward_cl(self, z_cl, head=None):
+        return convstack.run_stack(z_cl, self._plan, convstack.plan_params(self._owners), self._norms, head=head)
 
     def forward(self, z):
         y = self.forward_cl(convstack._LayoutIn.apply(z))
diff --git a/lvt_amd/modeling/loss/loss.py b/lvt_amd/modeling/loss/loss.py
--- a/lvt_amd/modeling/loss/loss.py
+++ b/lvt_amd/modeling/loss/loss.py
@@ -37,3 +37,6 @@
 
     def forward(self, input, target, denom=None):
         return self._fn(input, target, denom, self._lambda)
+
+    def head(self, target, denom=None):
+        return (target.contiguous(), float(denom if denom is not None else target.numel()), self._lambda, self._fn is l1)
diff --git a/lvt_amd/modeling/meta_arch/vqvae.py b/lvt_amd/modeling/meta_arch/vqvae.py
--- a/lvt_amd/modeling/meta_arch/vqvae.py
+++ b/lvt_amd/modeling/meta_arch/vqvae.py
@@ -70,16 +70,22 @@
     def _supervised_loss_cl(self, x, return_x=False):
         z_e = self.encoder.forward_cl(x)
         z_q_st = self.codebook.straight_through_cl(z_e, defer=True)
+        c = len(self.cfg.MODEL.PIXEL_MEAN)
         try:
-            x_tilde = self.generator.forward_cl(z_q_st)
+            x_tilde, reconstruction = self.generator.forward_cl(
+                z_q_st, head=self.pixel_loss.head(x, denom=x.numel() // x.shape[-1] * c))
         except BaseException:
             self.codebook.abandon_ema()
             raise
-        z_q_bar = self.codebook.finish_ema()
-        c = len(self.cfg.MODEL.PIXEL_MEAN)
+        if self.use_codebook_ema and isinstance(self.codebook, DVQEmbedding):
+            self.codebook.finish_ema(want_bar=False)
+            commitment = self.codebook.commitment_loss(z_e, self.beta)
+        else:
+            z_q_bar = self.codebook.finish_ema()
+            commitment = mse(z_e, z_q_bar.detach(), scale=self.beta)
         loss = {
-            "loss_reconstruction": self.pixel_loss(x_tilde, x, denom=x.numel() // x.shape[-1] * c),
-            "loss_commitment": mse(z_e, z_q_bar.detach(), scale=self.beta),
+            "loss_reconstruction": reconstruction,
+            "loss_commitment": commitment,
         }
         if not self.use_codebook_ema:
             loss["loss_dict"] = mse(z_q_bar, z_e.detach())
diff --git a/lvt_amd/modeling/vq/vq_embedding.py b/lvt_amd/modeling/vq/vq_embedding.py
--- a/lvt_amd/modeling/vq/vq_embedding.py
+++ b/lvt_amd/modeling/vq/vq_embedding.py
@@ -1,3 +1,5 @@
+import weakref
+
 import torch
 from torch import nn
 
@@ -91,6 +93,13 @@
             self.register_buffer("running_sum", self.embedding.weight.detach().clone())
 
 
+class _PassLink:
+    __slots__ = ("idx", "w", "bar", "denom", "scale", "done", "__weakref__")
+
+    def __init__(self, idx, w):
+        self.idx, self.w, self.bar, self.denom, self.scale, self.done = idx, w, None, None, None, False
+
+
 class _StraightThroughFn(torch.autograd.Function):
 
     @staticmethod
@@ -103,12 +112,36 @@
         if owner.ema:
             stats, work, cand = owner._accumulate(idx, z2d, P, False)
         owner._pending = (idx, stats, work, cand)
+        ctx.link = owner._new_link(idx, w)
+        ctx.save_for_backward(z2d)
+        ctx.set_materialize_grads(False)
+        handle = torch.empty(1, dtype=torch.float32, device=z2d.device)
         ctx.mark_non_differentiable(idx)
-        return z_q_st, idx
-
-    @staticmethod
-    def backward(ctx, g_st, g_idx):
-        return g_st, None, None
+        return z_q_st, idx, handle
+
+    @staticmethod
+    def backward(ctx, g_st, g_idx, g_commit):
+        link = ctx.link
+        link.done = True
+        if g_commit is None or link.scale is None:
+            return g_st, None, None
+        (z2d,) = ctx.saved_tensors
+        add = g_st.contiguous() if g_st is not None else None
+        gout = g_commit.contiguous().view(1)
+        if link.bar is not None:
+            return ew.mse_bwd(z2d, link.bar, link.denom, link.scale, gout=gout, add=add), None, None
+        return vq.commit_bwd(z2d, link.idx, link.w, link.denom, link.scale, gout=gout, add=add), None, None
+
+
+class _CommitFn(torch.autograd.Function):
+
+    @staticmethod
+    def forward(ctx, handle, link, z2d):
+        return vq.commit_fwd(z2d, link.idx, link.w, link.denom, link.scale)
+
+    @staticmethod
+    def backward(ctx, g):
+        return g.contiguous().view(1), None, None
 
 
 class _GatherWithGradFn(torch.autograd.Function):
@@ -253,6 +286,7 @@
         self.decay, self.eps = 0.99, 1e-5
         self.ve = nn.ModuleList([VQEmbedding(K, D // num, ema) for _ in range(num)])
         self._flat_w = self._flat_rs = self._flat_rsum = None
+        self._handle, self._links = None, []
 
     def _flat(self):
         w0 = self.ve[0].embedding.weight
@@ -288,13 +322,18 @@
         L.require(z_cl)
         if getattr(self, "_pending", None) is not None:
             raise L.LvtError("DVQEmbedding: the EMA update of the previous pass was never finished (finish_ema)")
-        z_q_st, idx = _StraightThroughFn.apply(z_cl.view(n * h * w, d), self, h * w)
+        z_q_st, idx, self._handle = _StraightThroughFn.apply(z_cl.view(n * h * w, d), self, h * w)
         self.last_indices = idx.view(n, self.num, h, w)
         self._pending_shape = (n, 1, h, w, d)
         z_q_st = z_q_st.view(n, 1, h, w, d)
         return z_q_st if defer else (z_q_st, self.finish_ema())
 
-    def finish_ema(self):
+    def _new_link(self, idx, w):
+        link = _PassLink(idx, w)
+        self._links = [r for r in getattr(self, "_links", ()) if r() is not None and not r().done] + [weakref.ref(link)]
+        return link
+
+    def finish_ema(self, want_bar=True):
         pend = getattr(self, "_pending", None)
         if pend is None:
             raise L.LvtError("DVQEmbedding.finish_ema without a pending straight_through_cl")
@@ -304,12 +343,46 @@
         if stats is not None:
             if work is not None:
                 work.wait()
+            for r in getattr(self, "_links", ())[:-1]:
+                prev = r()
+                if prev is not None and prev.scale is not None and not prev.done and prev.bar is None and prev.w is w:
+                    prev.bar = vq.gather(prev.idx, w)
             self._finalize(stats, cand, rsize, rsum, w)
         if not self.ema:
+            self._handle = None
             return _GatherWithGradFn.apply(idx, self, *[v.embedding.weight for v in self.ve]).view(*self._pending_shape)
+        if not want_bar:
+            return None
+        self._handle = None
         return vq.gather(idx, w).view(*self._pending_shape)
 
+    def z_q_bar_cl(self):
+        n, num, h, w = self.last_indices.shape
+        return vq.gather(self.last_indices.view(n, num, h * w), self._flat()[0]).view(n, 1, h, w, self.D)
+
+    def commitment_loss(self, z_cl, scale=1.0):
+        from ..loss.loss import mse
+        if not self.ema:
+            raise L.LvtError("commitment_loss: a trained codebook's z_q_bar carries a gradient (finish_ema returns it)")
+        if getattr(self, "_pending", None) is not None:
+            raise L.LvtError("commitment_loss before finish_ema: the codebook is still the pre-update one")
+        n, _, h, w, d = z_cl.shape
+        L.require(z_cl)
+        z2d = z_cl.view(n * h * w, d)
+        idx = self.last_indices.view(n, self.num, h * w)
+        handle, self._handle = getattr(self, "_handle", None), None
+        if not (torch.is_grad_enabled() and z_cl.requires_grad):
+            return vq.commit_fwd(z2d.detach(), idx, self._flat()[0], z2d.numel(), scale)
+        link = handle.grad_fn.link if handle is not None and handle.grad_fn is not None else None
+        z_saved = handle.grad_fn.saved_tensors[0] if link is not None else None
+        if (link is None or link.scale is not None or link.done or link.idx.data_ptr() != idx.data_ptr()
+                or z_saved.data_ptr() != z2d.data_ptr() or z_saved.shape != z2d.shape):
+            return mse(z_cl, self.z_q_bar_cl(), scale=scale)
+        link.denom, link.scale = float(z2d.numel()), scale
+        return _CommitFn.apply(handle, link, z2d.detach())
+
     def abandon_ema(self):
+        self._handle = None
         pend = getattr(self, "_pending", None)
         if pend is not None:
             self._pending = None
```
